# theovincent/iS-DQN

Hardware: AMD Instinct MI355X
Metric: gradient-steps/sec (batch=256, K=9, 84x84x4) (higher is better)
Workload: dtype bf16x3 (split-bf16 MFMA operands hi+lo, fp32 accumulate)

## Files before the change

is-dqn_amd/build.py:

```python
import os
import subprocess
import sys

HERE = os.path.dirname(os.path.abspath(__file__))
CSRC = os.path.join(HERE, "csrc")
LIBDIR = os.path.join(HERE, "lib")
LIB = os.path.join(LIBDIR, "libisdqn_hip.so")
SOURCES = ["api.hip", "tree_kernels.hip", "replay_kernels.hip", "net_kernels.hip"]
HEADERS = sorted(f for f in os.listdir(os.path.join(os.path.dirname(os.path.abspath(__file__)), "csrc")) if f.endswith(".h")) + [
    os.path.join("..", "..", "include", "isdqn_hip.h")]
FLAGS = ["--offload-arch=gfx950", "-O3", "-fPIC", "-std=c++17", "-fno-gpu-rdc", "-ffp-contract=off", "-fno-slp-vectorize"]


def _stale(target, deps):
    if not os.path.exists(target):
        return True
    t = os.path.getmtime(target)
    return any(os.path.getmtime(d) > t for d in deps)


def build(force=False, verbose=True, variant=None, defines=(), extra_flags=()):
    hipcc = os.environ.get("HIPCC", "/opt/rocm/bin/hipcc")
    os.makedirs(LIBDIR, exist_ok=True)
    objdir = os.path.join(HERE, "build" if not variant else "build_" + variant)
    lib = LIB if not variant else os.path.join(LIBDIR, "libisdqn_hip_%s.so" % variant)
    flags = FLAGS + ["-D" + d for d in defines] + list(extra_flags)
    os.makedirs(objdir, exist_ok=True)
    headers = [os.path.join(CSRC, h) for h in HEADERS]
    objs = []
    procs = []
    for src in SOURCES:
        s = os.path.join(CSRC, src)
        o = os.path.join(objdir, src.replace(".hip", ".o"))
        objs.append(o)
        if force or _stale(o, [s] + headers):
            cmd = [hipcc] + flags + ["-c", s, "-o", o]
            if verbose:
                print(" ".join(cmd), flush=True)
            procs.append((src, subprocess.Popen(cmd)))
    failed = [src for src, p in procs if p.wait() != 0]
    if failed:
        raise RuntimeError(f"hipcc failed for {failed}")
    if force or procs or _stale(lib, objs):
        cmd = [hipcc, "--offload-arch=gfx950", "-shared", "-fPIC", "-o", lib] + objs
        if verbose:
            print(" ".join(cmd), flush=True)
        subprocess.check_call(cmd)
    return lib


def emit_asm(force=False, verbose=False):
    hipcc = os.environ.get("HIPCC", "/opt/rocm/bin/hipcc")
    objdir = os.path.join(HERE, "build")
    os.makedirs(objdir, exist_ok=True)
    headers = [os.path.join(CSRC, h) for h in HEADERS]
    outs, procs = [], []
    for src in SOURCES:
        s = os.path.join(CSRC, src)
        o = os.path.join(objdir, src.replace(".hip", ".s"))
        outs.append(o)
        if force or _stale(o, [s] + headers + [os.path.abspath(__file__)]):
            cmd = [hipcc] + [f for f in FLAGS if f != "-fPIC"] + ["-S", "--cuda-device-only", "-w", s, "-o", o]
            if verbose:
                print(" ".join(cmd), flush=True)
            procs.append((src, subprocess.Popen(cmd)))
    failed = [src for src, p in procs if p.wait() != 0]
    if failed:
        raise RuntimeError(f"hipcc -S failed for {failed}")
    return outs


if __name__ == "__main__":
    _variant = None
    _defs = []
    for _i, _a in enumerate(sys.argv):
        if _a == "--variant":
            _variant = sys.argv[_i + 1]
        if _a.startswith("-D"):
            _defs.append(_a[2:])
    _extra = [_a for _a in sys.argv[1:] if _a.startswith("-f") or _a.startswith("-m")]
    print(build(force="--force" in sys.argv, variant=_variant, defines=_defs, extra_flags=_extra))
    if "--emit-asm" in sys.argv:
        print("\n".join(emit_asm(force="--force" in sys.argv, verbose=True)))
```

is-dqn_amd/csrc/conv_img.h:

```cpp
#pragma once
#include "net_problems.h"

namespace isdqn {

__device__ __forceinline__ int column_slot(int c16) { return c16 < 4 ? 8 + c16 : (c16 < 12 ? c16 - 4 : c16); }
struct PixelOrder {
    int strips;
    int n_full;
    int full_w;
    FastDiv d_h8, d_rem, d_w;
    PixelOrder() : strips(0), n_full(0), full_w(0) {}
    PixelOrder(int H, int W, bool use_strips) : strips(use_strips ? 1 : 0), n_full(H * 8 * (W / 8)), full_w(8 * (W / 8)) {
        d_h8 = FastDiv((uint32_t)(H * 8));
        d_rem = FastDiv((uint32_t)(W % 8 ? W % 8 : 1));
        d_w = FastDiv((uint32_t)W);
    }
    __device__ __forceinline__ void map(int n, int& y, int& x) const {
        uint32_t a, b;
        if (!strips) {
            d_w.divmod((uint32_t)n, a, b);
            y = (int)a; x = (int)b;
        } else if (n < n_full) {
            d_h8.divmod((uint32_t)n, a, b);
            y = (int)(b >> 3); x = (int)(a * 8 + (b & 7));
        } else {
            d_rem.divmod((uint32_t)(n - n_full), a, b);
            y = (int)a; x = full_w + (int)b;
        }
    }
};

struct ConvImgParams {
    ConvGeom g;
    MatSrc W;
    const float* in;
    FrameSrc fs;
    const float *bias, *gamma, *beta;
    float scale;
    float* act;
    float* z;
    int n_img, z_img;
    int tiles_per_img;
    int R, Wp;
    int PP;
    int plane_elems;
    int ablate;
    FastDiv d_chunk, d_Wp, d_R;
    PixelOrder order;
    long long* stamps;
};

template <int MT, int PASSES, bool U8>
struct ConvImgTraits {
    static constexpr int BM = MT * 16;
    static constexpr int A_PLANES = PASSES >= 2 ? 2 : 1;
    static constexpr int B_PLANES = (PASSES >= 3) ? 2 : 1;
    struct GA {
        static constexpr int PITCH = 48;
        static constexpr int ELEMS = BM * PITCH;
        static constexpr int CHUNKS = BM * (GEMM_BK / 8);
    };
    static constexpr int A_STAGE = A_PLANES * GA::ELEMS;
};

__device__ __forceinline__ void xcd_image_tile(int wg, int n_img, int T, int& j, int& tile) {
    const int full = (n_img / 8) * 8 * T;
    if (T > 1 && wg < full) {
        const int grp = wg / (8 * T), r = wg - grp * 8 * T;
        j = grp * 8 + (r & 7);
        tile = r >> 3;
    } else {
        j = wg / T;
        tile = wg - j * T;
    }
}

template <int NTHR, int PLANES, int BATCH>
__device__ __forceinline__ void fill_image_s8(__bf16* img, int plane_elems, const float* src, int H, int W, int C, int y0, int x0,
                                              int Rl, int Wl, int PP, int tid, const FastDiv& d_cpp, const FastDiv& d_Wl) {
    const int cpp = C >> 3, n_chunks = Rl * Wl * cpp;
    uint32_t pix_u, cc_u, lr_u, xl_u;
    d_cpp.divmod((uint32_t)tid, pix_u, cc_u);
    d_Wl.divmod(pix_u, lr_u, xl_u);
    int cc = (int)cc_u, lr = (int)lr_u, xl = (int)xl_u, pix = (int)pix_u;
    uint32_t dpix_u, dcc_u, dpy_u, dpx_u;
    d_cpp.divmod((uint32_t)NTHR, dpix_u, dcc_u);
    d_Wl.divmod(dpix_u, dpy_u, dpx_u);
    const int dpix = (int)dpix_u, dcc = (int)dcc_u, dpy = (int)dpy_u, dpx = (int)dpx_u;
    for (int c0 = tid; c0 - tid < n_chunks; ) {
        float v[BATCH][8];
        int dst[BATCH];
#pragma unroll
        for (int u = 0; u < BATCH; ++u) {
            const bool on = c0 < n_chunks;
            const int iy = y0 + lr, ix = x0 + xl;
            const bool ok = on && iy >= 0 && iy < H && ix >= 0 && ix < W;
            load8_aligned(ok ? src + ((iy * W + ix) * C + cc * 8) : zero_chunk(), v[u]);
            dst[u] = on ? pix * PP + cc * 8 : -1;
            c0 += NTHR;
            cc += dcc;
            const int carry_c = cc >= cpp ? 1 : 0;
            cc -= carry_c ? cpp : 0;
            pix += dpix + carry_c;
            xl += dpx + carry_c;
            lr += dpy;
            const int carry_x = xl >= Wl ? 1 : 0;
            xl -= carry_x ? Wl : 0;
            lr += carry_x;
        }
#pragma unroll
        for (int u = 0; u < BATCH; ++u) {
            bf16x8 hi, lo;
            if constexpr (PLANES >= 2) {
                s8_unpack(v[u], hi, lo);
                if (dst[u] >= 0) *reinterpret_cast<bf16x8*>(img + plane_elems + dst[u]) = lo;
            } else {
                s8_unpack_hi(v[u], hi);
            }
            if (dst[u] >= 0) *reinterpret_cast<bf16x8*>(img + dst[u]) = hi;
        }
    }
}

template <int N>
struct ImagePrefetch {
    float v[N][8];
    int dst[N];
};
template <int NTHR, int N>
__device__ __forceinline__ void request_image_s8(ImagePrefetch<N>& r, const float* src, int H, int W, int C, int y0, int x0, int Rl, int Wl,
                                                 int PP, int tid, const FastDiv& d_cpp, const FastDiv& d_Wl) {
    const int cpp = C >> 3, n_chunks = Rl * Wl * cpp;
    uint32_t pix_u, cc_u, lr_u, xl_u;
    d_cpp.divmod((uint32_t)tid, pix_u, cc_u);
    d_Wl.divmod(pix_u, lr_u, xl_u);
    int cc = (int)cc_u, lr = (int)lr_u, xl = (int)xl_u, pix = (int)pix_u;
    uint32_t dpix_u, dcc_u, dpy_u, dpx_u;
    d_cpp.divmod((uint32_t)NTHR, dpix_u, dcc_u);
    d_Wl.divmod(dpix_u, dpy_u, dpx_u);
    const int dpix = (int)dpix_u, dcc = (int)dcc_u, dpy = (int)dpy_u, dpx = (int)dpx_u;
    int c0 = tid;
#pragma unroll
    for (int u = 0; u < N; ++u) {
        const bool on = c0 < n_chunks;
        const int iy = y0 + lr, ix = x0 + xl;
        const bool ok = on && iy >= 0 && iy < H && ix >= 0 && ix < W;
        load8_aligned(ok ? src + ((iy * W + ix) * C + cc * 8) : zero_chunk(), r.v[u]);
        r.dst[u] = on ? pix * PP + cc * 8 : -1;
        c0 += NTHR;
        cc += dcc;
        const int carry_c = cc >= cpp ? 1 : 0;
        cc -= carry_c ? cpp : 0;
        pix += dpix + carry_c;
        xl += dpx + carry_c;
        lr += dpy;
        const int carry_x = xl >= Wl ? 1 : 0;
        xl -= carry_x ? Wl : 0;
        lr += carry_x;
    }
}
template <int PLANES, int N>
__device__ __forceinline__ void commit_image_s8(__bf16* img, int plane_elems, const ImagePrefetch<N>& r) {
#pragma unroll
    for (int u = 0; u < N; ++u) {
        bf16x8 hi, lo;
        if constexpr (PLANES >= 2) {
            s8_unpack(r.v[u], hi, lo);
            if (r.dst[u] >= 0) *reinterpret_cast<bf16x8*>(img + plane_elems + r.dst[u]) = lo;
        } else {
            s8_unpack_hi(r.v[u], hi);
        }
        if (r.dst[u] >= 0) *reinterpret_cast<bf16x8*>(img + r.dst[u]) = hi;
    }
}

template <int NTHR, int STACK_MAX = 4>
__device__ __forceinline__ void fill_frames_u8(__bf16* img, const FrameSrc& fs, int j, int row_base, int x0, int R, int Wp, int tid,
                                               const FastDiv& d_cpr) {
    constexpr int PB = 2;
    const int cpr = Wp / 8, per_plane = R * cpr, plane = R * Wp;
    const uint8_t* base[STACK_MAX];
#pragma unroll
    for (int c = 0; c < STACK_MAX; ++c) {
        const int id = c < fs.stack ? fs.frame_id(j, c) : -1;
        base[c] = id >= 0 ? fs.frames + (int64_t)id * fs.stride : nullptr;
    }
    const uint8_t* zeros = reinterpret_cast<const uint8_t*>(zero_chunk());
    for (int pb = 0; pb < per_plane; pb += NTHR * PB) {
        unsigned long long raw[PB][STACK_MAX];
        int sh[PB], dst[PB];
#pragma unroll
        for (int k = 0; k < PB; ++k) {
            const int pos = pb + k * NTHR + tid;
            const bool on = pos < per_plane;
            uint32_t lr, cx;
            d_cpr.divmod((uint32_t)(on ? pos : 0), lr, cx);
            const int iy = row_base + (int)lr, ix0 = (int)cx * 8 + x0;
            const bool ok = on && iy >= 0 && iy < fs.H && ix0 > -8 && ix0 < fs.W;
            const int ixc = min(max(ix0, 0), fs.W - 8);
            const int off = iy * fs.W + ixc;
            sh[k] = ix0 - ixc;
            dst[k] = on ? (int)lr * Wp + (int)cx * 8 : -1;
#pragma unroll
            for (int c = 0; c < STACK_MAX; ++c)
                raw[k][c] = load_u64_unaligned((ok && base[c] != nullptr) ? base[c] + off : zeros);
        }
#pragma unroll
        for (int k = 0; k < PB; ++k)
#pragma unroll
            for (int c = 0; c < STACK_MAX; ++c) {
                if (c >= fs.stack) continue;
                float v[8];
                FrameSrc::patch8_cvt(raw[k][c], sh[k], v);
                bf16x8 hi;
                round8(v, hi);
                if (dst[k] >= 0) *reinterpret_cast<bf16x8*>(img + c * plane + dst[k]) = hi;
            }
    }
}


template <int MT, int PASSES, bool U8, int KG = 1>
__global__ __launch_bounds__(GEMM_THREADS * KG, (U8 && MT == 2 && PASSES == 2) ? 4 : 1) void conv_fwd_img_kernel(const ConvImgParams p) {
    ISDQN_EMPTY_KERNEL_RETURN
    using T = ConvImgTraits<MT, PASSES, U8>;
    using GA = typename T::GA;
    constexpr int NT = 2;
    constexpr int NTHR = GEMM_THREADS;
    constexpr int NTHR_ALL = GEMM_THREADS * KG;
    constexpr int MTW = MT;
    extern __shared__ __attribute__((aligned(16))) char smem_raw[];
    __bf16* smem = reinterpret_cast<__bf16*>(smem_raw);
    const int tid_all = threadIdx.x, kg = KG > 1 ? tid_all / GEMM_THREADS : 0;
    __bf16* a_stage = smem + kg * 2 * T::A_STAGE;
    __bf16* img = smem + KG * 2 * T::A_STAGE;
    const ConvGeom& g = p.g;

    const int tid = tid_all - kg * GEMM_THREADS, lane = tid & 63, wave = tid >> 6;
#if defined(ISDQN_DEV)
#define ISDQN_STAMP(i)                                                                               \
    if (p.stamps != nullptr && threadIdx.x == 0) {                                                  \
        p.stamps[(int64_t)blockIdx.x * 8 + (i)] = (long long)__builtin_amdgcn_s_memtime();           \
        if ((i) == 0) p.stamps[(int64_t)blockIdx.x * 8 + 7] = (long long)__builtin_amdgcn_s_memrealtime(); \
    }
#define ISDQN_ABLATED(bit) ((p.ablate & (bit)) != 0)
#else
#define ISDQN_STAMP(i)
#define ISDQN_ABLATED(bit) (false)
#endif
    ISDQN_STAMP(0);
    if (ISDQN_ABLATED(8)) return;
    constexpr int mt0 = 0;
    int j, tile;
    xcd_image_tile((int)blockIdx.x, p.n_img, p.tiles_per_img, j, tile);
    const int p0 = tile * 128;
    const int oy_min = (int)g.d_wout.div((uint32_t)p0);
    const int row_base = oy_min * g.stride - g.pad;

    const int grp = lane >> 4;
    __shared__ __attribute__((aligned(16))) float s_par[3][64];
    float par_v = 0.f;
    {
        const int which = tid >> 6, ch = tid & 63;
        const float* src = which == 0 ? p.bias : which == 1 ? p.gamma : p.beta;
        const bool ok = kg == 0 && tid < 192 && ch < g.cout_p && src != nullptr;
        ISDQN_BOUNDS_CHECK(ok ? src + ch : zero_chunk(), 4, 13);
        par_v = *(const ISDQN_GLOBAL float*)(ok ? src + ch : zero_chunk());
    }

    const int nsteps = (g.K + GEMM_BK - 1) / GEMM_BK;
    const int k_last = g.K - 8;
    constexpr int A_PER = (GA::CHUNKS + NTHR - 1) / NTHR;
    int a_row[A_PER], a_var[A_PER], a_lds[A_PER];
    bool a_on[A_PER];
#pragma unroll
    for (int i = 0; i < A_PER; ++i) {
        int c = tid + i * NTHR;
        a_on[i] = c < GA::CHUNKS;
        if (!a_on[i]) c = 0;
        a_row[i] = stash_row(c);
        a_var[i] = (c & 3) * 8;
        a_lds[i] = a_row[i] * GA::PITCH + (c & 3) * 8;
    }
    constexpr int PF = 4;
    float sa[PF][A_PER][8];
    auto fetch = [&](int slot, int k) {
#pragma unroll
        for (int i = 0; i < A_PER; ++i) p.W.load(a_row[i], k + a_var[i], sa[slot][i]);
    };
    auto stash = [&](int slot, int stage) {
        __bf16* a_hi = a_stage + stage * T::A_STAGE;
        __bf16* a_lo = a_hi + GA::ELEMS;
#pragma unroll
        for (int i = 0; i < A_PER; ++i) {
            if (GA::CHUNKS % NTHR != 0 && !a_on[i]) continue;
            bf16x8 hi, lo;
            if constexpr (PASSES >= 2) {
                s8_unpack(sa[slot][i], hi, lo);
                *reinterpret_cast<bf16x8*>(a_lo + a_lds[i]) = lo;
            } else {
                s8_unpack_hi(sa[slot][i], hi);
            }
            *reinterpret_cast<bf16x8*>(a_hi + a_lds[i]) = hi;
        }
    };

    const int nsteps_p = ((nsteps + KG - 1) / KG + PF - 1) / PF * PF;
    const int rot = ISDQN_ABLATED(16) ? 0 : (int)((blockIdx.x >> 3) % (unsigned)nsteps);
    auto slice = [&](int s) {
        const int gs = s * KG + kg;
        const int k = gs + rot;
        return gs < nsteps ? (k >= nsteps ? k - nsteps : k) : nsteps_p * KG;
    };
#pragma unroll
    for (int d = 0; d < PF; ++d) fetch(d, slice(d) * GEMM_BK);

    constexpr int FILL_BATCH = (U8 ? 8 : 12) / KG;
    if (ISDQN_ABLATED(1)) {
    } else if constexpr (U8) {
#if defined(ISDQN_DEV)
        if (ISDQN_ABLATED(32)) {
            FrameSrc direct = p.fs;
            direct.ids = nullptr;
            fill_frames_u8<NTHR_ALL>(img, direct, j, row_base, -g.pad, p.R, p.Wp, tid_all, p.d_chunk);
        } else
#endif
        fill_frames_u8<NTHR_ALL>(img, p.fs, j, row_base, -g.pad, p.R, p.Wp, tid_all, p.d_chunk);
    } else {
        fill_image_s8<NTHR_ALL, T::B_PLANES, FILL_BATCH>(img, p.plane_elems, p.in + (int64_t)j * g.hin * g.win * g.cin_p, g.hin, g.win,
                                                         g.cin_p, row_base, -g.pad, p.R, p.Wp, p.PP, tid_all, p.d_chunk, p.d_Wp);
    }

    ISDQN_STAMP(1);
    int b_org[NT];
    int out_pix[NT];
#pragma unroll
    for (int nt = 0; nt < NT; ++nt) {
        int pp = p0 + wave * 32 + nt * 16 + (U8 ? (lane & 15) : column_slot(lane & 15));
        const bool in_img = pp < g.npix;
        pp = in_img ? pp : g.npix - 1;
        int oy, ox;
        if constexpr (U8) {
            uint32_t oy_u, ox_u;
            g.d_wout.divmod((uint32_t)pp, oy_u, ox_u);
            oy = (int)oy_u; ox = (int)ox_u;
        } else {
            p.order.map(pp, oy, ox);
        }
        out_pix[nt] = in_img ? oy * g.wout + ox : -1;
        const int ly0 = oy * g.stride - g.pad - row_base;
        const int lx0 = ox * g.stride;
        b_org[nt] = U8 ? (ly0 * p.Wp + lx0) : (ly0 * p.Wp + lx0) * p.PP;
    }

    f32x4 acc[MTW][NT];
#pragma unroll
    for (int mt = 0; mt < MTW; ++mt)
#pragma unroll
        for (int nt = 0; nt < NT; ++nt) mfma_init(acc[mt][nt]);


    struct Frags {
        bf16x8 a_hi[MTW], a_lo[MTW], b_hi[NT], b_lo[NT];
    };
    auto read_frags = [&](int stage, int kk, Frags& f) {
        const __bf16* a_hi = a_stage + stage * T::A_STAGE;
        const __bf16* a_lo = a_hi + GA::ELEMS;
#pragma unroll
        for (int mt = 0; mt < MTW; ++mt) {
            f.a_hi[mt] = read_frag<false, GA::PITCH>(a_hi, (mt0 + mt) * 16, lane);
            if constexpr (PASSES >= 2) f.a_lo[mt] = read_frag<false, GA::PITCH>(a_lo, (mt0 + mt) * 16, lane);
        }
        int kq = kk * GEMM_BK + grp * 8;
        kq = kq < k_last ? kq : k_last;
        int tap_off;
        if constexpr (U8) {
            const int c = kq >> 6, ky = (kq >> 3) & 7;
            tap_off = (c * p.R + ky) * p.Wp;
        } else {
            uint32_t tap, ci, ky, kx;
            g.d_cinp.divmod((uint32_t)kq, tap, ci);
            g.d_ksz.divmod(tap, ky, kx);
            tap_off = ((int)ky * p.Wp + (int)kx) * p.PP + (int)ci;
        }
#pragma unroll
        for (int nt = 0; nt < NT; ++nt) {
            const __bf16* src = img + b_org[nt] + tap_off;
            if constexpr (U8) {
                typedef __attribute__((ext_vector_type(4))) __bf16 bf16x4;
                bf16x4 h0 = *reinterpret_cast<const bf16x4*>(src);
                bf16x4 h1 = *reinterpret_cast<const bf16x4*>(src + 4);
                f.b_hi[nt] = __builtin_shufflevector(h0, h1, 0, 1, 2, 3, 4, 5, 6, 7);
            } else {
                f.b_hi[nt] = *reinterpret_cast<const bf16x8*>(src);
                if constexpr (PASSES >= 3) f.b_lo[nt] = *reinterpret_cast<const bf16x8*>(src + p.plane_elems);
            }
        }
    };
    auto mfma_step = [&](const Frags& f) {
#pragma unroll
        for (int nt = 0; nt < NT; ++nt)
#pragma unroll
            for (int mt = 0; mt < MTW; ++mt) {
                if constexpr (PASSES >= 3)
                    mfma_acc(acc[mt][nt], f.a_hi[mt], f.b_lo[nt]);
                if constexpr (PASSES >= 2)
                    mfma_acc(acc[mt][nt], f.a_lo[mt], f.b_hi[nt]);
                mfma_acc(acc[mt][nt], f.a_hi[mt], f.b_hi[nt]);
            }
    };

    static_assert(PF % 2 == 0 && PF >= 4, "the fragment sets alternate with the step parity; steps 0..3 are pre-fetched");
    Frags fr[2];
    if (kg == 0 && tid < 192) s_par[tid >> 6][tid & 63] = par_v;
    stash(0, 0);
    stash(1, 1);
    fetch(0, slice(PF) * GEMM_BK);
    fetch(1, slice(PF + 1) * GEMM_BK);
    __syncthreads();
    ISDQN_STAMP(2);
    if (!ISDQN_ABLATED(2)) {
        read_frags(0, slice(0), fr[0]);
        __syncthreads();
        constexpr bool INTERLEAVED = !U8 && PASSES == 3 && MTW == 4 && NT == 2 && A_PER == 1 &&
                                     GA::CHUNKS == NTHR;
        auto tap_offset_of = [&](int kk) {
            int kq = kk * GEMM_BK + grp * 8;
            kq = kq < k_last ? kq : k_last;
            uint32_t tap, ci, ky, kx;
            g.d_cinp.divmod((uint32_t)kq, tap, ci);
            g.d_ksz.divmod(tap, ky, kx);
            return ((int)ky * p.Wp + (int)kx) * p.PP + (int)ci;
        };
        int tap_next = INTERLEAVED ? tap_offset_of(slice(1)) : 0;
        for (int s0 = 0; s0 < nsteps_p; s0 += PF) {
#pragma unroll
            for (int u = 0; u < PF; ++u) {
                const int s = s0 + u;
                if constexpr (INTERLEAVED) {
                    const Frags& fc = fr[u & 1];
                    Frags& fn = fr[(u + 1) & 1];
                    const __bf16* na_hi = a_stage + ((s + 1) & 1) * T::A_STAGE;
                    const __bf16* na_lo = na_hi + GA::ELEMS;
                    const int tap_off = tap_next;
                    const int slot = (u + 2) % PF;
                    __bf16* st_hi = a_stage + (s & 1) * T::A_STAGE + a_lds[0];
                    __bf16* st_lo = st_hi + GA::ELEMS;
                    bf16x8 c_hi, c_lo;
                    __builtin_amdgcn_sched_barrier(0);
#pragma unroll
                    for (int j = 0; j < 24; ++j) {
                        const int pass = j >> 3, nt = (j >> 2) & 1, mt = j & 3;
                        mfma_acc(acc[mt][nt], pass == 1 ? fc.a_lo[mt] : fc.a_hi[mt], pass == 0 ? fc.b_lo[nt] : fc.b_hi[nt]);
                        if (j < 4) fn.a_hi[j] = read_frag<false, GA::PITCH>(na_hi, j * 16, lane);
                        else if (j < 8) fn.a_lo[j - 4] = read_frag<false, GA::PITCH>(na_lo, (j - 4) * 16, lane);
                        else if (j < 10) fn.b_hi[j - 8] = *reinterpret_cast<const bf16x8*>(img + b_org[j - 8] + tap_off);
                        else if (j < 12) fn.b_lo[j - 10] = *reinterpret_cast<const bf16x8*>(img + b_org[j - 10] + tap_off + p.plane_elems);
                        else if (j == 12) s8_unpack(sa[slot][0], c_hi, c_lo);
                        else if (j < 16) {
                        } else if (j == 16) *reinterpret_cast<bf16x8*>(st_lo) = c_lo;
                        else if (j == 17) *reinterpret_cast<bf16x8*>(st_hi) = c_hi;
                        else if (j == 18) fetch(slot, slice(s + 2 + PF) * GEMM_BK);
                        else if (j == 19) tap_next = tap_offset_of(slice(s + 2));
                        __builtin_amdgcn_sched_barrier(0);
                    }
                    __syncthreads();
                    continue;
                }
                read_frags((s + 1) & 1, slice(s + 1), fr[(u + 1) & 1]);
                mfma_step(fr[u & 1]);
                stash((u + 2) % PF, s & 1);
                fetch((u + 2) % PF, slice(s + 2 + PF) * GEMM_BK);
                constexpr int N_MFMA = MTW * NT * (PASSES >= 3 ? 3 : PASSES);
#pragma unroll
                for (int i = 0; i < N_MFMA; ++i) {
                    __builtin_amdgcn_sched_group_barrier(0x008, 1, 0);
                    if (i < N_MFMA / 2) __builtin_amdgcn_sched_group_barrier(0x100, 1, 0);
                    __builtin_amdgcn_sched_group_barrier(0x002, 2, 0);
                }
                __syncthreads();
            }
        }
    }
    ISDQN_STAMP(3);
    if constexpr (KG > 1) {
        static_assert(KG == 2 && NT == 2, "one pixel tile per K group");
        float* red = reinterpret_cast<float*>(img);
#pragma unroll
        for (int mt = 0; mt < MTW; ++mt)
#pragma unroll
            for (int r = 0; r < 4; ++r) {
                const float give = kg == 0 ? acc[mt][1][r] : acc[mt][0][r];
                red[(((kg * 4 + wave) * MTW + mt) * 4 + r) * 64 + lane] = give;
            }
        __syncthreads();
#pragma unroll
        for (int mt = 0; mt < MTW; ++mt)
#pragma unroll
            for (int r = 0; r < 4; ++r) {
                const float got = red[((((1 - kg) * 4 + wave) * MTW + mt) * 4 + r) * 64 + lane];
                if (kg == 0) acc[mt][0][r] += got;
                else acc[mt][1][r] += got;
            }
    }
    if (ISDQN_ABLATED(4)) {
        if (acc[0][0][0] == 12345.678f) p.act[0] = 1.f;
        return;
    }

    float bi[MTW][4], ga[MTW][4], be[MTW][4];
#pragma unroll
    for (int mt = 0; mt < MTW; ++mt) {
        const int ch0 = ((mt0 + mt) * 16 + grp * 4) & 63;
        const float4 b4 = *reinterpret_cast<const float4*>(&s_par[0][ch0]);
        const float4 g4 = *reinterpret_cast<const float4*>(&s_par[1][ch0]);
        const float4 e4 = *reinterpret_cast<const float4*>(&s_par[2][ch0]);
        bi[mt][0] = b4.x; bi[mt][1] = b4.y; bi[mt][2] = b4.z; bi[mt][3] = b4.w;
        ga[mt][0] = g4.x; ga[mt][1] = g4.y; ga[mt][2] = g4.z; ga[mt][3] = g4.w;
        be[mt][0] = e4.x; be[mt][1] = e4.y; be[mt][2] = e4.z; be[mt][3] = e4.w;
    }
    const float inv_c = 1.0f / (float)g.cout;
    float zv[NT][MTW][4], s1[NT], s2[NT];
#pragma unroll
    for (int nt = 0; nt < NT; ++nt) {
        s1[nt] = s2[nt] = 0.f;
        if (KG > 1 && nt != kg) continue;
#pragma unroll
        for (int mt = 0; mt < MTW; ++mt)
#pragma unroll
            for (int r = 0; r < 4; ++r) {
                int ch = (mt0 + mt) * 16 + grp * 4 + r;
                float zz = ch < g.cout ? acc[mt][nt][r] * p.scale + bi[mt][r] : 0.f;
                zv[nt][mt][r] = zz;
                s1[nt] += zz;
                s2[nt] += zz * zz;
            }
        if (p.gamma != nullptr) {
            s1[nt] += __shfl_xor(s1[nt], 16); s1[nt] += __shfl_xor(s1[nt], 32);
            s2[nt] += __shfl_xor(s2[nt], 16); s2[nt] += __shfl_xor(s2[nt], 32);
        }
    }
#pragma unroll
    for (int nt = 0; nt < NT; ++nt) {
        if (KG > 1 && nt != kg) continue;
        float mean = 0.f, rstd = 1.f;
        if (p.gamma != nullptr) {
            mean = s1[nt] * inv_c;
            float var = fmaxf(s2[nt] * inv_c - mean * mean, 0.f);
            rstd = rsqrtf(var + 1e-6f);
        }
        if (out_pix[nt] >= 0) {
            const int64_t pix = (int64_t)j * g.npix + out_pix[nt];
#pragma unroll
            for (int mt = 0; mt < MTW; ++mt) {
                int ch0 = (mt0 + mt) * 16 + grp * 4;
                if (ch0 >= g.cout_p) continue;
                float4 a, zq;
                float* ap = &a.x;
                float* zp = &zq.x;
#pragma unroll
                for (int r = 0; r < 4; ++r) {
                    float y = p.gamma != nullptr ? (zv[nt][mt][r] - mean) * (rstd * ga[mt][r]) + be[mt][r] : zv[nt][mt][r];
                    ap[r] = (ch0 + r < g.cout) ? fmaxf(y, 0.f) : 0.f;
                    zp[r] = zv[nt][mt][r];
                }
                s8_store_quad_paired(p.act + pix * g.cout_p, ch0, a.x, a.y, a.z, a.w);
                if (j < p.z_img) *reinterpret_cast<float4*>(p.z + pix * g.cout_p + ch0) = zq;
            }
        }
    }
    ISDQN_STAMP(4);
#if defined(ISDQN_DEV)
    if (p.stamps != nullptr) {
        __builtin_amdgcn_s_waitcnt(0);
        ISDQN_STAMP(5);
    }
#endif
#undef ISDQN_STAMP
#undef ISDQN_ABLATED
}

template <int MT, int PASSES, bool U8, int KG = 1>
static int launch_conv_fwd_img(const ConvImgParams& p, hipStream_t st) {
    using T = ConvImgTraits<MT, PASSES, U8>;
    const int lds = (KG * 2 * T::A_STAGE + T::B_PLANES * p.plane_elems) * 2;
    static LdsConfigured configured;
    if (int rc = ensure_dynamic_lds(&conv_fwd_img_kernel<MT, PASSES, U8, KG>, lds, configured)) return rc;
    ISDQN_REPORT_OCCUPANCY((&conv_fwd_img_kernel<MT, PASSES, U8, KG>), GEMM_THREADS * KG, lds, p.n_img * p.tiles_per_img);
    hipLaunchKernelGGL((conv_fwd_img_kernel<MT, PASSES, U8, KG>), dim3(p.n_img * p.tiles_per_img), dim3(GEMM_THREADS * KG), lds,
                       st, p);
    ISDQN_HIP_CHECK(hipGetLastError());
    return ISDQN_OK;
}

static inline int conv_img_geometry(const ConvGeom& g, bool u8, int stack, int b_planes, int mt, int a_planes, int& R,
                                    int& Wp, int& plane_elems, int pixel_pitch = 0) {
    int rows_per_tile = g.npix <= 128 ? g.hout : ((128 + g.wout - 2) / g.wout + 1);
    if (rows_per_tile > g.hout) rows_per_tile = g.hout;
    R = g.stride * (rows_per_tile - 1) + g.ksz;
    if (u8) {
        Wp = ((g.wout - 1) * g.stride + g.ksz + 7) / 8 * 8;
        plane_elems = stack * R * Wp;
    } else {
        Wp = (g.wout - 1) * g.stride + g.ksz;
        plane_elems = R * Wp * (pixel_pitch ? pixel_pitch : g.cin_p);
    }
    const int a_stage = a_planes * (mt * 16) * 48;
    return (2 * a_stage + b_planes * plane_elems) * 2;
}


struct ConvWgradImgParams {
    ConvGeom g;
    const float* dz;
    const float* in;
    FrameSrc fs;
    float* slabs;
    float scale;
    int n_img, G;
    int n_col_groups, NC;
    int R, Wp;
    int PPin;
    int in_plane;
    int PA, npix_pad;
    int dz_plane;
    FastDiv d_ncg;
    FastDiv d_chunk, d_Wp, d_R, d_dzchunk, d_npixpad;
    int prefetch;
    long long* stamps;
};
template <int WV> struct WgradPrefetch { static constexpr int DZ = 1024 / (64 * WV), IN = WV == 4 ? 6 : 5, DZ_U8 = 1792 / (64 * WV); };

template <bool U8, int PASSES, int NTHR = GEMM_THREADS>
__device__ __forceinline__ void fill_input_image(__bf16* img, int plane_elems, const ConvGeom& g, const FrameSrc& fs,
                                                 const float* in, int j, int row_base, int R, int Wp, int PP, int tid,
                                                 const FastDiv& d_chunk, const FastDiv& d_Wp, const FastDiv& d_R) {
    constexpr int FILL_BATCH = 8;
    if constexpr (U8) {
        fill_frames_u8<NTHR>(img, fs, j, row_base, -g.pad, R, Wp, tid, d_chunk);
    } else {
        fill_image_s8<NTHR, (PASSES >= 3 ? 2 : 1), FILL_BATCH>(img, plane_elems, in + (int64_t)j * g.hin * g.win * g.cin_p, g.hin, g.win, g.cin_p,
                                                               row_base, -g.pad, R, Wp, PP, tid, d_chunk, d_Wp);
    }
}

__device__ __forceinline__ bf16x8 tr_frag(const __bf16* a0, const __bf16* a1) {
    s16x4 lo = __builtin_amdgcn_ds_read_tr16_b64_v4i16((LDS_AS s16x4*)a0);
    s16x4 hi = __builtin_amdgcn_ds_read_tr16_b64_v4i16((LDS_AS s16x4*)a1);
    s16x8 r = __builtin_shufflevector(lo, hi, 0, 1, 2, 3, 4, 5, 6, 7);
    return __builtin_bit_cast(bf16x8, r);
}

template <int MT, int NTW, int PASSES, bool U8, int WV = 4>
__global__ __launch_bounds__(64 * WV) void conv_wgrad_img_kernel(const ConvWgradImgParams p) {
    ISDQN_EMPTY_KERNEL_RETURN
    constexpr int NTHR = 64 * WV;
    constexpr int A_PLANES = PASSES >= 2 ? 2 : 1;
    constexpr int B_PLANES = (PASSES >= 3) ? 2 : 1;
    extern __shared__ __attribute__((aligned(16))) char smem_raw[];
    __bf16* dzi = reinterpret_cast<__bf16*>(smem_raw);
    __bf16* img = dzi + A_PLANES * p.dz_plane;
    const ConvGeom& g = p.g;
    const int tid = threadIdx.x, lane = tid & 63, wave = tid >> 6;
#if defined(ISDQN_DEV)
#define WG_STAMP(i)                                                                                   \
    if (p.stamps != nullptr && threadIdx.x == 0) {                                                   \
        p.stamps[(int64_t)blockIdx.x * 8 + (i)] = (long long)__builtin_amdgcn_s_memtime();            \
        if ((i) == 0) p.stamps[(int64_t)blockIdx.x * 8 + 7] = (long long)__builtin_amdgcn_s_memrealtime(); \
    }
#else
#define WG_STAMP(i)
#endif
    WG_STAMP(0);
    uint32_t ig_u, cg_u;
    p.d_ncg.divmod(blockIdx.x, ig_u, cg_u);
    const int cg = (int)cg_u, ig = (int)ig_u;
    const int j0 = ig * p.G, j1 = min(p.n_img, j0 + p.G);
    const int grp = lane >> 4, li = lane & 15, q = li >> 2, pq = li & 3;

    int col_off[NTW];
#pragma unroll
    for (int t = 0; t < NTW; ++t) {
        const int c0 = cg * p.NC + (wave + WV * t) * 16;
        if constexpr (U8) {
            const int c = c0 >> 6, ky0 = (c0 >> 3) & 7;
            col_off[t] = (c * p.R + ky0 + (pq >> 1)) * p.Wp + 4 * (pq & 1);
        } else {
            uint32_t tap, ci, ky, kx;
            g.d_cinp.divmod((uint32_t)(c0 < g.K ? c0 : 0), tap, ci);
            g.d_ksz.divmod(tap, ky, kx);
            col_off[t] = ((int)ky * p.Wp + (int)kx) * p.PPin + (int)ci + 4 * pq;
        }
    }

    f32x4 acc[MT][NTW];
#pragma unroll
    for (int mt = 0; mt < MT; ++mt)
#pragma unroll
        for (int t = 0; t < NTW; ++t) mfma_init(acc[mt][t]);

    const int nsteps = p.npix_pad / GEMM_BK;
    auto k_steps = [&]() {
        for (int ks = 0; ks < nsteps; ++ks) {
            int pixoff[2], arow[2];
#pragma unroll
            for (int h = 0; h < 2; ++h) {
                int kp = ks * GEMM_BK + tr_row(8 * grp + 4 * h + q);
                arow[h] = kp * p.PA + 4 * pq;
                kp = kp < g.npix ? kp : g.npix - 1;
                uint32_t oy, ox;
                g.d_wout.divmod((uint32_t)kp, oy, ox);
                pixoff[h] = U8 ? ((int)oy * g.stride * p.Wp + (int)ox * g.stride)
                               : ((int)oy * g.stride * p.Wp + (int)ox * g.stride) * p.PPin;
            }
            bf16x8 fa_hi[MT], fa_lo[MT];
#pragma unroll
            for (int mt = 0; mt < MT; ++mt) {
                fa_hi[mt] = tr_frag(dzi + arow[0] + mt * 16, dzi + arow[1] + mt * 16);
                if constexpr (PASSES >= 2)
                    fa_lo[mt] = tr_frag(dzi + p.dz_plane + arow[0] + mt * 16, dzi + p.dz_plane + arow[1] + mt * 16);
            }
#pragma unroll
            for (int t = 0; t < NTW; ++t) {
                const __bf16* b0 = img + pixoff[0] + col_off[t];
                const __bf16* b1 = img + pixoff[1] + col_off[t];
                bf16x8 fb_hi = tr_frag(b0, b1), fb_lo;
                if constexpr (PASSES >= 3) fb_lo = tr_frag(b0 + p.in_plane, b1 + p.in_plane);
#pragma unroll
                for (int mt = 0; mt < MT; ++mt) {
                    if constexpr (PASSES >= 3)
                        mfma_acc(acc[mt][t], fa_hi[mt], fb_lo);
                    if constexpr (PASSES >= 2)
                        mfma_acc(acc[mt][t], fa_lo[mt], fb_hi);
                    mfma_acc(acc[mt][t], fa_hi[mt], fb_hi);
                }
            }
        }
    };
    bool staged = false;
    if constexpr (!U8) {
        if (p.prefetch) {
            staged = true;
            ImagePrefetch<WgradPrefetch<WV>::DZ> ra;
            ImagePrefetch<WgradPrefetch<WV>::IN> rb;
            auto request = [&](int j) {
                request_image_s8<NTHR>(ra, p.dz + (int64_t)j * g.npix * g.cout_p, 1, g.npix, g.cout_p, 0, 0, 1, p.npix_pad, p.PA, tid,
                                       p.d_dzchunk, p.d_npixpad);
                request_image_s8<NTHR>(rb, p.in + (int64_t)j * g.hin * g.win * g.cin_p, g.hin, g.win, g.cin_p, -g.pad, -g.pad, p.R, p.Wp,
                                       p.PPin, tid, p.d_chunk, p.d_Wp);
            };
            request(j0);
            for (int j = j0; j < j1; ++j) {
                __syncthreads();
                commit_image_s8<A_PLANES>(dzi, p.dz_plane, ra);
                commit_image_s8<B_PLANES>(img, p.in_plane, rb);
                __syncthreads();
                if (j == j0) { WG_STAMP(1); } else if (j == j0 + 1) { WG_STAMP(3); }
                if (j + 1 < j1) request(j + 1);
                k_steps();
                if (j == j0) { WG_STAMP(2); } else if (j == j0 + 1) { WG_STAMP(4); }
            }
        }
    }
    if (!staged)
    for (int j = j0; j < j1; ++j) {
        __syncthreads();
        bool dz_done = false;
        if constexpr (U8) {
            if (p.prefetch) {
                ImagePrefetch<WgradPrefetch<WV>::DZ_U8> ra;
                request_image_s8<NTHR>(ra, p.dz + (int64_t)j * g.npix * g.cout_p, 1, g.npix, g.cout_p, 0, 0, 1, p.npix_pad, p.PA, tid,
                                       p.d_dzchunk, p.d_npixpad);
                fill_input_image<U8, PASSES, NTHR>(img, p.in_plane, g, p.fs, p.in, j, -g.pad, p.R, p.Wp, p.PPin, tid, p.d_chunk, p.d_Wp, p.d_R);
                commit_image_s8<A_PLANES>(dzi, p.dz_plane, ra);
                dz_done = true;
            }
        }
        if (!dz_done) {
            fill_image_s8<NTHR, A_PLANES, 8>(dzi, p.dz_plane, p.dz + (int64_t)j * g.npix * g.cout_p, 1, g.npix, g.cout_p, 0, 0, 1, p.npix_pad,
                                             p.PA, tid, p.d_dzchunk, p.d_npixpad);
            fill_input_image<U8, PASSES, NTHR>(img, p.in_plane, g, p.fs, p.in, j, -g.pad, p.R, p.Wp, p.PPin, tid, p.d_chunk, p.d_Wp, p.d_R);
        }
        __syncthreads();
        if (j == j0) { WG_STAMP(1); } else if (j == j0 + 1) { WG_STAMP(3); }
        k_steps();
        if (j == j0) { WG_STAMP(2); } else if (j == j0 + 1) { WG_STAMP(4); }
    }

    float* slab = p.slabs + (int64_t)ig * g.cout_p * g.K;
#pragma unroll
    for (int mt = 0; mt < MT; ++mt)
#pragma unroll
        for (int t = 0; t < NTW; ++t) {
            const int col = cg * p.NC + (wave + WV * t) * 16 + li;
#pragma unroll
            for (int r = 0; r < 4; ++r) {
                const int row = mt * 16 + grp * 4 + r;
#if !defined(ISDQN_NO_STREAMING)
                if (row < g.cout_p && col < g.K) __builtin_nontemporal_store(acc[mt][t][r] * p.scale, (ISDQN_GLOBAL float*)(slab + (int64_t)row * g.K + col));
#else
                if (row < g.cout_p && col < g.K) slab[(int64_t)row * g.K + col] = acc[mt][t][r] * p.scale;
#endif
            }
        }
#if defined(ISDQN_DEV)
    if (p.stamps != nullptr) {
        __builtin_amdgcn_s_waitcnt(0);
        WG_STAMP(5);
    }
#endif
#undef WG_STAMP
}

template <int MT, int NTW, int PASSES, bool U8, int WV = 4>
static int launch_conv_wgrad_img(const ConvWgradImgParams& p, int n_img_groups, hipStream_t st) {
    constexpr int A_PLANES = PASSES >= 2 ? 2 : 1;
    constexpr int B_PLANES = (PASSES >= 3) ? 2 : 1;
    const int lds = (A_PLANES * p.dz_plane + B_PLANES * p.in_plane) * 2;
    static LdsConfigured configured;
    if (int rc = ensure_dynamic_lds(&conv_wgrad_img_kernel<MT, NTW, PASSES, U8, WV>, lds, configured)) return rc;
    ISDQN_REPORT_OCCUPANCY((&conv_wgrad_img_kernel<MT, NTW, PASSES, U8, WV>), 64 * WV, lds, n_img_groups * p.n_col_groups);
    ConvWgradImgParams q = p;
    q.prefetch = 0;
#if !defined(ISDQN_WGRAD_NO_PREFETCH)
    if (!U8 && p.G >= 2 && p.npix_pad * (p.g.cout_p / 8) <= WgradPrefetch<WV>::DZ * 64 * WV &&
        p.R * p.Wp * (p.g.cin_p / 8) <= WgradPrefetch<WV>::IN * 64 * WV)
        q.prefetch = 1;
#if !defined(ISDQN_WGRAD_NO_U8_DZ)
    if (U8 && p.npix_pad * (p.g.cout_p / 8) <= WgradPrefetch<WV>::DZ_U8 * 64 * WV) q.prefetch = 1;
#endif
#endif
    hipLaunchKernelGGL((conv_wgrad_img_kernel<MT, NTW, PASSES, U8, WV>), dim3(n_img_groups * p.n_col_groups),
                       dim3(64 * WV), lds, st, q);
    ISDQN_HIP_CHECK(hipGetLastError());
    return ISDQN_OK;
}


struct ConvDgradImgParams {
    ConvGeom g;
    const float* W;
    const float* dz;
    const float* z_in;
    const float *gamma, *beta;
    int c_in;
    float* dz_in;
    float* part;
    int n_img, T, Kc;
    int Hd, Wd, PPd, bt;
    FastDiv d_chunk, d_Wd, d_T;
    long long* stamps;
    int dz_plane;
    int tiles_per_img;
    int cls_tile_start[5];
    PixelOrder cls_order[4];
    int n_classes;
};

template <int MT, int PASSES, int NT = 2>
__global__ __launch_bounds__(GEMM_THREADS, 2) void conv_dgrad_img_kernel(const ConvDgradImgParams p) {
    ISDQN_EMPTY_KERNEL_RETURN
    constexpr int BM = MT * 16;
    constexpr int A_PLANES = PASSES >= 2 ? 2 : 1;
    constexpr int B_PLANES = PASSES >= 3 ? 2 : 1;
    using GA = TileGeom<BM, true>;
    constexpr int A_STAGE = A_PLANES * GA::ELEMS;
    extern __shared__ __attribute__((aligned(16))) char smem_raw[];
    __bf16* a_stage = reinterpret_cast<__bf16*>(smem_raw);
    __bf16* img = a_stage + 2 * A_STAGE;
    __shared__ float s_part[4][3][64];
    const ConvGeom& g = p.g;
    const int tid = threadIdx.x, lane = tid & 63, wave = tid >> 6, grp = lane >> 4;
#if defined(ISDQN_DEV)
#define ISDQN_STAMP(i)                                                                               \
    if (p.stamps != nullptr && threadIdx.x == 0) {                                                  \
        p.stamps[(int64_t)blockIdx.x * 8 + (i)] = (long long)__builtin_amdgcn_s_memtime();           \
        if ((i) == 0) p.stamps[(int64_t)blockIdx.x * 8 + 7] = (long long)__builtin_amdgcn_s_memrealtime(); \
    }
#define ISDQN_ABLATED(bit) ((p.ablate & (bit)) != 0)
#else
#define ISDQN_STAMP(i)
#define ISDQN_ABLATED(bit) (false)
#endif
    ISDQN_STAMP(0);

    int j, tl;
    xcd_image_tile((int)blockIdx.x, p.n_img, p.tiles_per_img, j, tl);
    int cls = 0;
    while (cls + 1 < p.n_classes && tl >= p.cls_tile_start[cls + 1]) ++cls;
    const int q0 = (tl - p.cls_tile_start[cls]) * (64 * NT);
    const int smask = g.stride - 1;
    const int cy = cls >> g.stride_sh, cx = cls & smask;
    const int Ha = (g.hin - cy + g.stride - 1) >> g.stride_sh, Wb = (g.win - cx + g.stride - 1) >> g.stride_sh;
    const int n_cls_pix = Ha * Wb;
    const int py = (cy + g.pad) & smask, px = (cx + g.pad) & smask;

    __shared__ __attribute__((aligned(16))) float s_gb[2][64];
    float par_v = 0.f;
    {
        const int which = tid >> 6, ch = tid & 63;
        const float* src = which == 0 ? p.gamma : p.beta;
        const bool ok = tid < 128 && ch < g.cin_p && p.gamma != nullptr;
        ISDQN_BOUNDS_CHECK(ok ? src + ch : zero_chunk(), 4, 13);
        par_v = *(const ISDQN_GLOBAL float*)(ok ? src + ch : zero_chunk());
    }

    const int nsteps = (p.Kc + GEMM_BK - 1) / GEMM_BK;
    const int k_last = p.Kc - 8;
    constexpr int A_PER = GA::PER_THREAD;
    int a_ci0[A_PER], a_kk[A_PER], a_lds[A_PER];
    bool a_on[A_PER];
#pragma unroll
    for (int i = 0; i < A_PER; ++i) {
        int c = tid + i * GEMM_THREADS;
        a_on[i] = c < GA::CHUNKS;
        if (!a_on[i]) c = 0;
        const int kk = c / (BM / 8), rc = c % (BM / 8);
        a_ci0[i] = rc * 8; a_kk[i] = kk;
        a_lds[i] = tr_row(kk) * GA::PITCH + rc * 8;
    }
    constexpr int PF = 4;
    float sa[PF][A_PER][8];
    auto fetch = [&](int slot, int k0) {
#pragma unroll
        for (int i = 0; i < A_PER; ++i) {
            const int k = k0 + a_kk[i];
            const bool ok = (k < p.Kc) && (a_ci0[i] < g.cin_p);
            uint32_t jt, co;
            g.d_coutp.divmod(ok ? (uint32_t)k : 0u, jt, co);
            uint32_t jy_u, jx_u;
            p.d_T.divmod(jt, jy_u, jx_u);
            const int jy = (int)jy_u, jx = (int)jx_u;
            const int ky = py + g.stride * jy, kx = px + g.stride * jx;
            load8_aligned(ok ? p.W + ((int64_t)co * g.K + (ky * g.ksz + kx) * g.cin_p + a_ci0[i]) : zero_chunk(), sa[slot][i]);
        }
    };
    auto stash = [&](int slot, int stage) {
        __bf16* a_hi = a_stage + stage * A_STAGE;
        __bf16* a_lo = a_hi + GA::ELEMS;
#pragma unroll
        for (int i = 0; i < A_PER; ++i) {
            if (GA::CHUNKS % GEMM_THREADS != 0 && !a_on[i]) continue;
            bf16x8 hi, lo;
            if constexpr (PASSES >= 2) {
                s8_unpack(sa[slot][i], hi, lo);
                *reinterpret_cast<bf16x8*>(a_lo + a_lds[i]) = lo;
            } else {
                s8_unpack_hi(sa[slot][i], hi);
            }
            *reinterpret_cast<bf16x8*>(a_hi + a_lds[i]) = hi;
        }
    };

    const int nsteps_p = (nsteps + PF - 1) / PF * PF;
    const int rot = (int)((blockIdx.x >> 3) % (unsigned)nsteps);
    auto slice = [&](int s) {
        const int k = s + rot;
        return s < nsteps ? (k >= nsteps ? k - nsteps : k) : nsteps_p;
    };
#pragma unroll
    for (int d = 0; d < PF; ++d) fetch(d, slice(d) * GEMM_BK);

    fill_image_s8<GEMM_THREADS, B_PLANES, 8>(img, p.dz_plane, p.dz + (int64_t)j * g.hout * g.wout * g.cout_p, g.hout, g.wout, g.cout_p,
                                             -p.bt, -p.bt, p.Hd, p.Wd, p.PPd, tid, p.d_chunk, p.d_Wd);

    ISDQN_STAMP(1);
    int b_org[NT], pix_iy[NT], pix_ix[NT];
    bool pix_ok[NT];
#pragma unroll
    for (int nt = 0; nt < NT; ++nt) {
        int q = q0 + wave * (16 * NT) + nt * 16 + column_slot(lane & 15);
        pix_ok[nt] = q < n_cls_pix;
        q = pix_ok[nt] ? q : n_cls_pix - 1;
        int a, b;
        p.cls_order[cls].map(q, a, b);
        const int iy = cy + g.stride * a, ix = cx + g.stride * b;
        pix_iy[nt] = iy; pix_ix[nt] = ix;
        const int oyb = (iy + g.pad - py) >> g.stride_sh, oxb = (ix + g.pad - px) >> g.stride_sh;
        b_org[nt] = ((oyb + p.bt) * p.Wd + oxb + p.bt) * p.PPd;
    }

    f32x4 acc[MT][NT];
#pragma unroll
    for (int mt = 0; mt < MT; ++mt)
#pragma unroll
        for (int nt = 0; nt < NT; ++nt) mfma_init(acc[mt][nt]);

    struct Frags {
        bf16x8 a_hi[MT], a_lo[MT], b_hi[NT], b_lo[NT];
    };
    auto read_frags = [&](int stage, int kk, Frags& f) {
        const __bf16* a_hi = a_stage + stage * A_STAGE;
        const __bf16* a_lo = a_hi + GA::ELEMS;
#pragma unroll
        for (int mt = 0; mt < MT; ++mt) {
            f.a_hi[mt] = read_frag<true, GA::PITCH>(a_hi, mt * 16, lane);
            if constexpr (PASSES >= 2) f.a_lo[mt] = read_frag<true, GA::PITCH>(a_lo, mt * 16, lane);
        }
        int kq = kk * GEMM_BK + grp * 8;
        kq = kq < k_last ? kq : k_last;
        uint32_t jt, co;
        g.d_coutp.divmod((uint32_t)kq, jt, co);
        uint32_t jy_u, jx_u;
        p.d_T.divmod(jt, jy_u, jx_u);
        const int jy = (int)jy_u, jx = (int)jx_u;
        const int tap_off = -(jy * p.Wd + jx) * p.PPd + (int)co;
#pragma unroll
        for (int nt = 0; nt < NT; ++nt) {
            const __bf16* src = img + b_org[nt] + tap_off;
            f.b_hi[nt] = *reinterpret_cast<const bf16x8*>(src);
            if constexpr (PASSES >= 3) f.b_lo[nt] = *reinterpret_cast<const bf16x8*>(src + p.dz_plane);
        }
    };
    auto mfma_step = [&](const Frags& f) {
#pragma unroll
        for (int nt = 0; nt < NT; ++nt)
#pragma unroll
            for (int mt = 0; mt < MT; ++mt) {
                if constexpr (PASSES >= 3)
                    mfma_acc(acc[mt][nt], f.a_hi[mt], f.b_lo[nt]);
                if constexpr (PASSES >= 2)
                    mfma_acc(acc[mt][nt], f.a_lo[mt], f.b_hi[nt]);
                mfma_acc(acc[mt][nt], f.a_hi[mt], f.b_hi[nt]);
            }
    };

    float zpre[NT][MT][4];
#pragma unroll
    for (int nt = 0; nt < NT; ++nt) {
        const int64_t pixel = ((int64_t)j * g.hin + pix_iy[nt]) * g.win + pix_ix[nt];
#pragma unroll
        for (int mt = 0; mt < MT; ++mt) {
            const int ch0 = mt * 16 + grp * 4;
            ISDQN_BOUNDS_CHECK(ch0 < g.cin_p ? p.z_in + pixel * g.cin_p + ch0 : zero_chunk(), 16, 12);
            const ISDQN_GLOBAL f32x4* zp = (const ISDQN_GLOBAL f32x4*)(ch0 < g.cin_p ? p.z_in + pixel * g.cin_p + ch0 : zero_chunk());
            const f32x4 zq = *zp;
            zpre[nt][mt][0] = zq[0]; zpre[nt][mt][1] = zq[1]; zpre[nt][mt][2] = zq[2]; zpre[nt][mt][3] = zq[3];
        }
    }

    static_assert(PF % 2 == 0 && PF >= 4, "the fragment sets alternate with the step parity; steps 0..3 are pre-fetched");
    Frags fr[2];
    if (tid < 128) s_gb[tid >> 6][tid & 63] = par_v;
    stash(0, 0);
    stash(1, 1);
    fetch(0, slice(PF) * GEMM_BK);
    fetch(1, slice(PF + 1) * GEMM_BK);
    __syncthreads();
    ISDQN_STAMP(2);
    read_frags(0, slice(0), fr[0]);
    __syncthreads();
    constexpr bool INTERLEAVED = PASSES == 3 && MT == 4 && A_PER == 1 && GA::CHUNKS == GEMM_THREADS;
    auto tap_offset_of = [&](int kk) {
        int kq = kk * GEMM_BK + grp * 8;
        kq = kq < k_last ? kq : k_last;
        uint32_t jt, co, jy_u, jx_u;
        g.d_coutp.divmod((uint32_t)kq, jt, co);
        p.d_T.divmod(jt, jy_u, jx_u);
        return -((int)jy_u * p.Wd + (int)jx_u) * p.PPd + (int)co;
    };
    int tap_next = INTERLEAVED ? tap_offset_of(slice(1)) : 0;
    for (int s0 = 0; s0 < nsteps_p; s0 += PF) {
#pragma unroll
        for (int u = 0; u < PF; ++u) {
            const int s = s0 + u;
            if constexpr (INTERLEAVED) {
                const Frags& fc = fr[u & 1];
                Frags& fn = fr[(u + 1) & 1];
                const __bf16* na_hi = a_stage + ((s + 1) & 1) * A_STAGE;
                const __bf16* na_lo = na_hi + GA::ELEMS;
                const int tap_off = tap_next;
                const int slot = (u + 2) % PF;
                __bf16* st_hi = a_stage + (s & 1) * A_STAGE + a_lds[0];
                __bf16* st_lo = st_hi + GA::ELEMS;
                bf16x8 c_hi, c_lo;
                constexpr int NM = 12 * NT;
                __builtin_amdgcn_sched_barrier(0);
#pragma unroll
                for (int jm = 0; jm < NM; ++jm) {
                    const int pass = jm / (4 * NT), nt = (jm >> 2) % NT, mt = jm & 3;
                    mfma_acc(acc[mt][nt], pass == 1 ? fc.a_lo[mt] : fc.a_hi[mt], pass == 0 ? fc.b_lo[nt] : fc.b_hi[nt]);
                    if (jm < 4) fn.a_hi[jm] = read_frag<true, GA::PITCH>(na_hi, jm * 16, lane);
                    else if (jm < 8) fn.a_lo[jm - 4] = read_frag<true, GA::PITCH>(na_lo, (jm - 4) * 16, lane);
                    else if (jm < 8 + NT) fn.b_hi[jm - 8] = *reinterpret_cast<const bf16x8*>(img + b_org[jm - 8] + tap_off);
                    else if (jm < 8 + 2 * NT) fn.b_lo[jm - 8 - NT] = *reinterpret_cast<const bf16x8*>(img + b_org[jm - 8 - NT] + tap_off + p.dz_plane);
                    else if constexpr (NT == 2) {
                        if (jm == 12) s8_unpack(sa[slot][0], c_hi, c_lo);
                        else if (jm == 16) *reinterpret_cast<bf16x8*>(st_lo) = c_lo;
                        else if (jm == 17) *reinterpret_cast<bf16x8*>(st_hi) = c_hi;
                        else if (jm == 18) fetch(slot, slice(s + 2 + PF) * GEMM_BK);
                        else if (jm == 19) tap_next = tap_offset_of(slice(s + 2));
                    } else {
                        if (jm == 10) {
                            s8_unpack(sa[slot][0], c_hi, c_lo);
                            *reinterpret_cast<bf16x8*>(st_lo) = c_lo;
                            *reinterpret_cast<bf16x8*>(st_hi) = c_hi;
                        } else if (jm == 11) {
                            fetch(slot, slice(s + 2 + PF) * GEMM_BK);
                            tap_next = tap_offset_of(slice(s + 2));
                        }
                    }
                    __builtin_amdgcn_sched_barrier(0);
                }
                __syncthreads();
                continue;
            }
            read_frags((s + 1) & 1, slice(s + 1), fr[(u + 1) & 1]);
            mfma_step(fr[u & 1]);
            stash((u + 2) % PF, s & 1);
            fetch((u + 2) % PF, slice(s + 2 + PF) * GEMM_BK);
            constexpr int N_MFMA = MT * NT * (PASSES >= 3 ? 3 : PASSES);
#pragma unroll
            for (int i = 0; i < N_MFMA; ++i) {
                __builtin_amdgcn_sched_group_barrier(0x008, 1, 0);
                if (i < N_MFMA / 2) __builtin_amdgcn_sched_group_barrier(0x100, 1, 0);
                __builtin_amdgcn_sched_group_barrier(0x002, 2, 0);
            }
            __syncthreads();
        }
    }

    ISDQN_STAMP(3);
    float ga[MT][4], be[MT][4];
#pragma unroll
    for (int mt = 0; mt < MT; ++mt) {
        const int ch0 = (mt * 16 + grp * 4) & 63;
        const float4 g4 = *reinterpret_cast<const float4*>(&s_gb[0][ch0]);
        const float4 e4 = *reinterpret_cast<const float4*>(&s_gb[1][ch0]);
        ga[mt][0] = g4.x; ga[mt][1] = g4.y; ga[mt][2] = g4.z; ga[mt][3] = g4.w;
        be[mt][0] = e4.x; be[mt][1] = e4.y; be[mt][2] = e4.z; be[mt][3] = e4.w;
    }
    float dg[MT][4], db[MT][4], dbias[MT][4];
#pragma unroll
    for (int mt = 0; mt < MT; ++mt)
#pragma unroll
        for (int r = 0; r < 4; ++r) dg[mt][r] = db[mt][r] = dbias[mt][r] = 0.f;
    const float inv_c = 1.f / (float)p.c_in;
#pragma unroll
    for (int nt = 0; nt < NT; ++nt) {
        const int64_t pixel = ((int64_t)j * g.hin + pix_iy[nt]) * g.win + pix_ix[nt];
        float zv[MT][4];
#pragma unroll
        for (int mt = 0; mt < MT; ++mt)
#pragma unroll
            for (int r = 0; r < 4; ++r) zv[mt][r] = zpre[nt][mt][r];
        float out[MT][4];
        if (p.gamma != nullptr) {
            float s1 = 0.f, s2 = 0.f;
#pragma unroll
            for (int mt = 0; mt < MT; ++mt)
#pragma unroll
                for (int r = 0; r < 4; ++r) {
                    const bool ok = (mt * 16 + grp * 4 + r) < p.c_in;
                    s1 += ok ? zv[mt][r] : 0.f;
                    s2 += ok ? zv[mt][r] * zv[mt][r] : 0.f;
                }
            s1 += __shfl_xor(s1, 16); s1 += __shfl_xor(s1, 32);
            s2 += __shfl_xor(s2, 16); s2 += __shfl_xor(s2, 32);
            const float mean = s1 * inv_c;
            const float rstd = rsqrtf(fmaxf(s2 * inv_c - mean * mean, 0.f) + 1e-6f);
            float xh[MT][4], gg[MT][4], m1 = 0.f, m2 = 0.f;
#pragma unroll
            for (int mt = 0; mt < MT; ++mt)
#pragma unroll
                for (int r = 0; r < 4; ++r) {
                    const bool ok = pix_ok[nt] && (mt * 16 + grp * 4 + r) < p.c_in;
                    xh[mt][r] = (zv[mt][r] - mean) * rstd;
                    const float y = xh[mt][r] * ga[mt][r] + be[mt][r];
                    const float dy = (ok && y > 0.f) ? acc[mt][nt][r] : 0.f;
                    dg[mt][r] += dy * xh[mt][r];
                    db[mt][r] += dy;
                    gg[mt][r] = dy * ga[mt][r];
                    m1 += gg[mt][r];
                    m2 += gg[mt][r] * xh[mt][r];
                }
            m1 += __shfl_xor(m1, 16); m1 += __shfl_xor(m1, 32);
            m2 += __shfl_xor(m2, 16); m2 += __shfl_xor(m2, 32);
            m1 *= inv_c;
            m2 *= inv_c;
#pragma unroll
            for (int mt = 0; mt < MT; ++mt)
#pragma unroll
                for (int r = 0; r < 4; ++r) {
                    const bool ok = pix_ok[nt] && (mt * 16 + grp * 4 + r) < p.c_in;
                    out[mt][r] = ok ? rstd * (gg[mt][r] - m1 - xh[mt][r] * m2) : 0.f;
                    dbias[mt][r] += out[mt][r];
                }
        } else {
#pragma unroll
            for (int mt = 0; mt < MT; ++mt)
#pragma unroll
                for (int r = 0; r < 4; ++r) {
                    const bool ok = pix_ok[nt] && (mt * 16 + grp * 4 + r) < p.c_in;
                    out[mt][r] = (ok && zv[mt][r] > 0.f) ? acc[mt][nt][r] : 0.f;
                    dbias[mt][r] += out[mt][r];
                }
        }
        if (pix_ok[nt]) {
#pragma unroll
            for (int mt = 0; mt < MT; ++mt) {
                const int ch0 = mt * 16 + grp * 4;
                if (ch0 < g.cin_p)
                    s8_store_quad_paired(p.dz_in + pixel * g.cin_p, ch0, out[mt][0], out[mt][1], out[mt][2], out[mt][3]);
            }
        }
    }
#pragma unroll
    for (int mt = 0; mt < MT; ++mt)
#pragma unroll
        for (int r = 0; r < 4; ++r) {
            dg[mt][r] = row16_sum(dg[mt][r]);
            db[mt][r] = row16_sum(db[mt][r]);
            dbias[mt][r] = row16_sum(dbias[mt][r]);
            if ((lane & 15) == 0) {
                const int ch = mt * 16 + grp * 4 + r;
                s_part[wave][0][ch] = dg[mt][r];
                s_part[wave][1][ch] = db[mt][r];
                s_part[wave][2][ch] = dbias[mt][r];
            }
        }
    __syncthreads();
    for (int i = tid; i < 3 * g.cin_p; i += GEMM_THREADS) {
        const int which = (i >= g.cin_p) + (i >= 2 * g.cin_p), c = i - which * g.cin_p;
        p.part[((int64_t)blockIdx.x * 3 + which) * g.cin_p + c] =
            s_part[0][which][c] + s_part[1][which][c] + s_part[2][which][c] + s_part[3][which][c];
    }
    ISDQN_STAMP(4);
#if defined(ISDQN_DEV)
    if (p.stamps != nullptr) {
        __builtin_amdgcn_s_waitcnt(0);
        ISDQN_STAMP(5);
    }
#endif
#undef ISDQN_STAMP
#undef ISDQN_ABLATED
}

constexpr int REDUCE_MAX_JOBS = 4;
struct ReduceJobs {
    const float* part[REDUCE_MAX_JOBS];
    float* out[REDUCE_MAX_JOBS];
    int n_rows[REDUCE_MAX_JOBS], width[REDUCE_MAX_JOBS];
    int block_start[REDUCE_MAX_JOBS + 1];
    int n;
};
__global__ __launch_bounds__(256) void reduce_rows_kernel(const ReduceJobs jobs) {
    ISDQN_EMPTY_KERNEL_RETURN
    __shared__ float s_red[32][8];
    int job = 0;
#pragma unroll
    for (int i = 1; i < REDUCE_MAX_JOBS; ++i)
        if (i < jobs.n && (int)blockIdx.x >= jobs.block_start[i]) job = i;
    const float* __restrict__ part = jobs.part[job];
    float* __restrict__ out = jobs.out[job];
    const int n_rows = jobs.n_rows[job], width = jobs.width[job];
    const int col = ((int)blockIdx.x - jobs.block_start[job]) * 8 + (threadIdx.x & 7), rl = threadIdx.x >> 3;
    float s = 0.f;
    if (col < width) {
        int r = rl;
        for (; r + 7 * 32 < n_rows; r += 8 * 32) {
            float v[8];
#pragma unroll
            for (int u = 0; u < 8; ++u) v[u] = part[(int64_t)(r + u * 32) * width + col];
#pragma unroll
            for (int u = 0; u < 8; ++u) s += v[u];
        }
        for (; r < n_rows; r += 32) s += part[(int64_t)r * width + col];
    }
    s_red[rl][threadIdx.x & 7] = s;
    __syncthreads();
    if (rl == 0 && col < width) {
        float t = 0.f;
#pragma unroll
        for (int k = 0; k < 32; ++k) t += s_red[k][threadIdx.x & 7];
        out[col] = t;
    }
}

template <int MT, int PASSES, int NT = 2>
static int launch_conv_dgrad_img(const ConvDgradImgParams& p, hipStream_t st) {
    constexpr int A_PLANES = PASSES >= 2 ? 2 : 1;
    constexpr int B_PLANES = PASSES >= 3 ? 2 : 1;
    using GA = TileGeom<MT * 16, true>;
    const int lds = (2 * A_PLANES * GA::ELEMS + B_PLANES * p.dz_plane) * 2;
    static LdsConfigured configured;
    if (int rc = ensure_dynamic_lds(&conv_dgrad_img_kernel<MT, PASSES, NT>, lds, configured)) return rc;
    ISDQN_REPORT_OCCUPANCY((&conv_dgrad_img_kernel<MT, PASSES, NT>), GEMM_THREADS, lds, p.n_img * p.tiles_per_img);
    hipLaunchKernelGGL((conv_dgrad_img_kernel<MT, PASSES, NT>), dim3(p.n_img * p.tiles_per_img), dim3(GEMM_THREADS), lds, st, p);
    ISDQN_HIP_CHECK(hipGetLastError());
    return ISDQN_OK;
}

}
```

is-dqn_amd/csrc/conv_s8_pair.h:

```cpp
#pragma once
#include "conv_img.h"

namespace isdqn {

constexpr int S8P_BATCH = 6;

template <int NPOS>
__global__ __launch_bounds__(GEMM_THREADS * 2, 1) void conv_fwd_s8_pair_kernel(const ConvImgParams p) {
    ISDQN_EMPTY_KERNEL_RETURN
    constexpr int MT = 4, PASSES = 3, KG = 2, NT = 2, MTW = MT, NTHR = GEMM_THREADS, NTHR_ALL = GEMM_THREADS * KG;
    using T = ConvImgTraits<MT, PASSES, false>;
    using GA = typename T::GA;
    extern __shared__ __attribute__((aligned(16))) char smem_raw[];
    __bf16* smem = reinterpret_cast<__bf16*>(smem_raw);
    const int tid_all = threadIdx.x, kg = tid_all / GEMM_THREADS;
    __bf16* a_stage = smem + kg * 2 * T::A_STAGE;
    __bf16* img = smem + KG * 2 * T::A_STAGE;
    const ConvGeom& g = p.g;
    const int tid = tid_all - kg * GEMM_THREADS, lane = tid & 63, wave = tid >> 6, grp = lane >> 4;
    const int row_base = -g.pad;

    __shared__ __attribute__((aligned(16))) float s_par[3][64];
    float par_v = 0.f;
    {
        const int which = tid >> 6, ch = tid & 63;
        const float* src = which == 0 ? p.bias : which == 1 ? p.gamma : p.beta;
        const bool ok = kg == 0 && tid < 192 && ch < g.cout_p && src != nullptr;
        ISDQN_BOUNDS_CHECK(ok ? src + ch : zero_chunk(), 4, 13);
        par_v = *(const ISDQN_GLOBAL float*)(ok ? src + ch : zero_chunk());
    }
    constexpr int nsteps = NPOS * KG;
    const int k_last = g.K - 8;
    static_assert(GA::CHUNKS == NTHR, "one weight chunk per thread and K step");
    const int a_row = stash_row(tid), a_var = (tid & 3) * 8, a_lds = a_row * GA::PITCH + (tid & 3) * 8;
    constexpr int PF = 4;
    static_assert(NPOS >= PF + 2, "ring of four slices + two staged ones");
    float sa[PF][1][8];
    auto fetch = [&](int slot, int k) { p.W.load(a_row, k + a_var, sa[slot][0]); };
    auto stash = [&](int slot, int stage) {
        __bf16* a_hi = a_stage + stage * T::A_STAGE;
        __bf16* a_lo = a_hi + GA::ELEMS;
        bf16x8 hi, lo;
        s8_unpack(sa[slot][0], hi, lo);
        *reinterpret_cast<bf16x8*>(a_lo + a_lds) = lo;
        *reinterpret_cast<bf16x8*>(a_hi + a_lds) = hi;
    };

    const int cpp = g.cin_p >> 3, n_chunks = p.R * p.Wp * cpp;
    uint32_t dpix_u, dcc_u, dpy_u, dpx_u;
    p.d_chunk.divmod((uint32_t)NTHR_ALL, dpix_u, dcc_u);
    p.d_Wp.divmod(dpix_u, dpy_u, dpx_u);
    const int dpix = (int)dpix_u, dcc = (int)dcc_u, dpy = (int)dpy_u, dpx = (int)dpx_u;
    float rv[S8P_BATCH][8];
    auto walk = [&](auto&& visit) {
        uint32_t pix_u, cc_u, lr_u, xl_u;
        p.d_chunk.divmod((uint32_t)tid_all, pix_u, cc_u);
        p.d_Wp.divmod(pix_u, lr_u, xl_u);
        int cc = (int)cc_u, lr = (int)lr_u, xl = (int)xl_u, pix = (int)pix_u, c0 = tid_all;
#pragma unroll
        for (int u = 0; u < S8P_BATCH; ++u) {
            visit(u, c0 < n_chunks, lr, xl, cc, pix);
            c0 += NTHR_ALL;
            cc += dcc;
            const int carry_c = cc >= cpp ? 1 : 0;
            cc -= carry_c ? cpp : 0;
            pix += dpix + carry_c;
            xl += dpx + carry_c;
            lr += dpy;
            const int carry_x = xl >= p.Wp ? 1 : 0;
            xl -= carry_x ? p.Wp : 0;
            lr += carry_x;
        }
    };
    auto request = [&](int j) {
        const float* src = p.in + (int64_t)j * g.hin * g.win * g.cin_p;
        walk([&](int u, bool on, int lr, int xl, int cc, int) {
            const int iy = row_base + lr, ix = xl - g.pad;
            const bool ok = on && iy >= 0 && iy < g.hin && ix >= 0 && ix < g.win;
            load8_aligned(ok ? src + ((iy * g.win + ix) * g.cin_p + cc * 8) : zero_chunk(), rv[u]);
        });
    };
    auto commit = [&]() {
        walk([&](int u, bool on, int, int, int cc, int pix) {
            bf16x8 hi, lo;
            s8_unpack(rv[u], hi, lo);
            if (on) {
                const int dst = pix * p.PP + cc * 8;
                *reinterpret_cast<bf16x8*>(img + p.plane_elems + dst) = lo;
                *reinterpret_cast<bf16x8*>(img + dst) = hi;
            }
        });
    };

    int b_org[NT], out_pix[NT];
#pragma unroll
    for (int nt = 0; nt < NT; ++nt) {
        int pp = wave * 32 + nt * 16 + column_slot(lane & 15);
        const bool in_img = pp < g.npix;
        pp = in_img ? pp : g.npix - 1;
        int oy, ox;
        p.order.map(pp, oy, ox);
        out_pix[nt] = in_img ? oy * g.wout + ox : -1;
        const int ly0 = oy * g.stride - g.pad - row_base;
        const int lx0 = ox * g.stride;
        b_org[nt] = (ly0 * p.Wp + lx0) * p.PP;
    }
    struct Frags {
        bf16x8 a_hi[MTW], a_lo[MTW], b_hi[NT], b_lo[NT];
    };

    auto do_image = [&](auto it_c) {
        constexpr int it = decltype(it_c)::value;
#if defined(ISDQN_PAIR_PLAIN_ORDER)
        const bool by_xcd = false;
#else
        const bool by_xcd = (p.n_img & 15) == 0;
#endif
        const int bx = (int)blockIdx.x;
        const int j_first = by_xcd ? ((bx >> 3) << 4) + (bx & 7) : 2 * bx;
        const int j_second = by_xcd ? j_first + 8 : j_first + 1;
        const int j = it == 0 ? j_first : j_second;
        const int rot = (int)((unsigned)(j >> 3) % (unsigned)nsteps);
        auto slice = [&](int s) {
            const int k = s * KG + kg + rot;
            return k >= nsteps ? k - nsteps : k;
        };
        auto tap_offset_of = [&](int kk) {
            int kq = kk * GEMM_BK + grp * 8;
            kq = kq < k_last ? kq : k_last;
            uint32_t tap, ci, ky, kx;
            g.d_cinp.divmod((uint32_t)kq, tap, ci);
            g.d_ksz.divmod(tap, ky, kx);
            return ((int)ky * p.Wp + (int)kx) * p.PP + (int)ci;
        };
#pragma unroll
        for (int d = 0; d < PF; ++d) fetch(d, slice(d) * GEMM_BK);
        if constexpr (it == 0) request(j);
        commit();

        f32x4 acc[MTW][NT];
#pragma unroll
        for (int mt = 0; mt < MTW; ++mt)
#pragma unroll
            for (int nt = 0; nt < NT; ++nt) mfma_init(acc[mt][nt]);
        Frags fr[2];
        if constexpr (it == 0) {
            if (kg == 0 && tid < 192) s_par[tid >> 6][tid & 63] = par_v;
        }
        stash(0, 0);
        stash(1, 1);
        fetch(0, slice(PF) * GEMM_BK);
        fetch(1, slice(PF + 1) * GEMM_BK);
        __syncthreads();
        {
            const __bf16* a_hi = a_stage;
            const __bf16* a_lo = a_hi + GA::ELEMS;
#pragma unroll
            for (int mt = 0; mt < MTW; ++mt) {
                fr[0].a_hi[mt] = read_frag<false, GA::PITCH>(a_hi, mt * 16, lane);
                fr[0].a_lo[mt] = read_frag<false, GA::PITCH>(a_lo, mt * 16, lane);
            }
            const int tap_off = tap_offset_of(slice(0));
#pragma unroll
            for (int nt = 0; nt < NT; ++nt) {
                const __bf16* src = img + b_org[nt] + tap_off;
                fr[0].b_hi[nt] = *reinterpret_cast<const bf16x8*>(src);
                fr[0].b_lo[nt] = *reinterpret_cast<const bf16x8*>(src + p.plane_elems);
            }
        }
        __syncthreads();
        int tap_next = tap_offset_of(slice(1));
#pragma unroll
        for (int s = 0; s < NPOS; ++s) {
            const Frags& fc = fr[s & 1];
            Frags& fn = fr[(s + 1) & 1];
            const __bf16* na_hi = a_stage + ((s + 1) & 1) * T::A_STAGE;
            const __bf16* na_lo = na_hi + GA::ELEMS;
            const int tap_off = tap_next;
            const int slot = (s + 2) % PF;
            __bf16* st_hi = a_stage + (s & 1) * T::A_STAGE + a_lds;
            __bf16* st_lo = st_hi + GA::ELEMS;
            const bool nxt = s + 1 < NPOS, stg = s + 2 < NPOS, ftc = s + 2 + PF < NPOS;
            bf16x8 c_hi, c_lo;
            __builtin_amdgcn_sched_barrier(0);
#pragma unroll
            for (int q = 0; q < 24; ++q) {
                const int pass = q >> 3, nt = (q >> 2) & 1, mt = q & 3;
                mfma_acc(acc[mt][nt], pass == 1 ? fc.a_lo[mt] : fc.a_hi[mt], pass == 0 ? fc.b_lo[nt] : fc.b_hi[nt]);
                if (q < 4) { if (nxt) fn.a_hi[q] = read_frag<false, GA::PITCH>(na_hi, q * 16, lane); }
                else if (q < 8) { if (nxt) fn.a_lo[q - 4] = read_frag<false, GA::PITCH>(na_lo, (q - 4) * 16, lane); }
                else if (q < 10) { if (nxt) fn.b_hi[q - 8] = *reinterpret_cast<const bf16x8*>(img + b_org[q - 8] + tap_off); }
                else if (q < 12) { if (nxt) fn.b_lo[q - 10] = *reinterpret_cast<const bf16x8*>(img + b_org[q - 10] + tap_off + p.plane_elems); }
                else if (q == 12) { if (stg) s8_unpack(sa[slot][0], c_hi, c_lo); }
                else if (q < 16) {
                } else if (q == 16) { if (stg) *reinterpret_cast<bf16x8*>(st_lo) = c_lo; }
                else if (q == 17) { if (stg) *reinterpret_cast<bf16x8*>(st_hi) = c_hi; }
                else if (q == 18) { if (ftc) fetch(slot, slice(s + 2 + PF) * GEMM_BK); }
                else if (q == 19) { if (s + 2 < NPOS) tap_next = tap_offset_of(slice(s + 2)); }
                __builtin_amdgcn_sched_barrier(0);
            }
            if constexpr (it == 0) {
                if (s == NPOS - 3) request(j_second);
            }
            __syncthreads();
        }
        {
            float* red = reinterpret_cast<float*>(img);
#pragma unroll
            for (int mt = 0; mt < MTW; ++mt)
#pragma unroll
                for (int r = 0; r < 4; ++r) {
                    const float give = kg == 0 ? acc[mt][1][r] : acc[mt][0][r];
                    red[(((kg * 4 + wave) * MTW + mt) * 4 + r) * 64 + lane] = give;
                }
            __syncthreads();
#pragma unroll
            for (int mt = 0; mt < MTW; ++mt)
#pragma unroll
                for (int r = 0; r < 4; ++r) {
                    const float got = red[((((1 - kg) * 4 + wave) * MTW + mt) * 4 + r) * 64 + lane];
                    if (kg == 0) acc[mt][0][r] += got;
                    else acc[mt][1][r] += got;
                }
        }
        float bi[MTW][4], ga[MTW][4], be[MTW][4];
#pragma unroll
        for (int mt = 0; mt < MTW; ++mt) {
            const int ch0 = (mt * 16 + grp * 4) & 63;
            const float4 b4 = *reinterpret_cast<const float4*>(&s_par[0][ch0]);
            const float4 g4 = *reinterpret_cast<const float4*>(&s_par[1][ch0]);
            const float4 e4 = *reinterpret_cast<const float4*>(&s_par[2][ch0]);
            bi[mt][0] = b4.x; bi[mt][1] = b4.y; bi[mt][2] = b4.z; bi[mt][3] = b4.w;
            ga[mt][0] = g4.x; ga[mt][1] = g4.y; ga[mt][2] = g4.z; ga[mt][3] = g4.w;
            be[mt][0] = e4.x; be[mt][1] = e4.y; be[mt][2] = e4.z; be[mt][3] = e4.w;
        }
        const float inv_c = 1.0f / (float)g.cout;
        float zv[NT][MTW][4], s1[NT], s2[NT];
#pragma unroll
        for (int nt = 0; nt < NT; ++nt) {
            s1[nt] = s2[nt] = 0.f;
            if (nt != kg) continue;
#pragma unroll
            for (int mt = 0; mt < MTW; ++mt)
#pragma unroll
                for (int r = 0; r < 4; ++r) {
                    int ch = mt * 16 + grp * 4 + r;
                    float zz = ch < g.cout ? acc[mt][nt][r] * p.scale + bi[mt][r] : 0.f;
                    zv[nt][mt][r] = zz;
                    s1[nt] += zz;
                    s2[nt] += zz * zz;
                }
            if (p.gamma != nullptr) {
                s1[nt] += __shfl_xor(s1[nt], 16); s1[nt] += __shfl_xor(s1[nt], 32);
                s2[nt] += __shfl_xor(s2[nt], 16); s2[nt] += __shfl_xor(s2[nt], 32);
            }
        }
#pragma unroll
        for (int nt = 0; nt < NT; ++nt) {
            if (nt != kg) continue;
            float mean = 0.f, rstd = 1.f;
            if (p.gamma != nullptr) {
                mean = s1[nt] * inv_c;
                float var = fmaxf(s2[nt] * inv_c - mean * mean, 0.f);
                rstd = rsqrtf(var + 1e-6f);
            }
            if (out_pix[nt] >= 0) {
                const int64_t pix = (int64_t)j * g.npix + out_pix[nt];
#pragma unroll
                for (int mt = 0; mt < MTW; ++mt) {
                    int ch0 = mt * 16 + grp * 4;
                    if (ch0 >= g.cout_p) continue;
                    float4 a, zq;
                    float* ap = &a.x;
                    float* zp = &zq.x;
#pragma unroll
                    for (int r = 0; r < 4; ++r) {
                        float y = p.gamma != nullptr ? (zv[nt][mt][r] - mean) * (rstd * ga[mt][r]) + be[mt][r] : zv[nt][mt][r];
                        ap[r] = (ch0 + r < g.cout) ? fmaxf(y, 0.f) : 0.f;
                        zp[r] = zv[nt][mt][r];
                    }
                    s8_store_quad_paired(p.act + pix * g.cout_p, ch0, a.x, a.y, a.z, a.w);
                    if (j < p.z_img) *reinterpret_cast<float4*>(p.z + pix * g.cout_p + ch0) = zq;
                }
            }
        }
        if constexpr (it == 0) __syncthreads();
    };
    do_image(std::integral_constant<int, 0>{});
    do_image(std::integral_constant<int, 1>{});
}

template <int NPOS>
static int launch_conv_fwd_s8_pair(const ConvImgParams& p, hipStream_t st) {
    using T = ConvImgTraits<4, 3, false>;
    const int lds = (2 * 2 * T::A_STAGE + T::B_PLANES * p.plane_elems) * 2;
    static LdsConfigured configured;
    if (int rc = ensure_dynamic_lds(&conv_fwd_s8_pair_kernel<NPOS>, lds, configured)) return rc;
    ISDQN_REPORT_OCCUPANCY((&conv_fwd_s8_pair_kernel<NPOS>), GEMM_THREADS * 2, lds, p.n_img / 2);
    hipLaunchKernelGGL((conv_fwd_s8_pair_kernel<NPOS>), dim3(p.n_img / 2), dim3(GEMM_THREADS * 2), lds, st, p);
    ISDQN_HIP_CHECK(hipGetLastError());
    return ISDQN_OK;
}

}
```

is-dqn_amd/csrc/conv_u8_pair.h:

```cpp
#pragma once
#include "conv_img.h"

namespace isdqn {

constexpr int U8P_PB = 2;

template <int PASSES, int NSTEPS>
__global__ __launch_bounds__(GEMM_THREADS, 4) void conv_fwd_u8_pair_kernel(const ConvImgParams p) {
    ISDQN_EMPTY_KERNEL_RETURN
    constexpr int MT = 2, NT = 2, MTW = MT, NTHR = GEMM_THREADS, STACK_MAX = 4;
    using T = ConvImgTraits<MT, PASSES, true>;
    using GA = typename T::GA;
    extern __shared__ __attribute__((aligned(16))) char smem_raw[];
    __bf16* smem = reinterpret_cast<__bf16*>(smem_raw);
    __bf16* a_stage = smem;
    __bf16* img = smem + 2 * T::A_STAGE;
    const ConvGeom& g = p.g;
    const int tid = threadIdx.x, lane = tid & 63, wave = tid >> 6, grp = lane >> 4;
#if defined(ISDQN_DEV)
#define U8P_STAMP(i)                                                                                 \
    if (p.stamps != nullptr && threadIdx.x == 0) {                                                  \
        p.stamps[(int64_t)blockIdx.x * 8 + (i)] = (long long)__builtin_amdgcn_s_memtime();           \
        if ((i) == 0) p.stamps[(int64_t)blockIdx.x * 8 + 7] = (long long)__builtin_amdgcn_s_memrealtime(); \
    }
#else
#define U8P_STAMP(i)
#endif
    U8P_STAMP(0);
    const int T2 = p.tiles_per_img >> 1;
    int j, tp;
    xcd_image_tile((int)blockIdx.x, p.n_img, T2, j, tp);

    __shared__ __attribute__((aligned(16))) float s_par[3][64];
    float par_v = 0.f;
    {
        const int which = tid >> 6, ch = tid & 63;
        const float* src = which == 0 ? p.bias : which == 1 ? p.gamma : p.beta;
        const bool ok = tid < 192 && ch < g.cout_p && src != nullptr;
        ISDQN_BOUNDS_CHECK(ok ? src + ch : zero_chunk(), 4, 13);
        par_v = *(const ISDQN_GLOBAL float*)(ok ? src + ch : zero_chunk());
    }
    constexpr int nsteps = NSTEPS;
    const int k_last = g.K - 8;
    constexpr int A_PER = (GA::CHUNKS + NTHR - 1) / NTHR;
    int a_row[A_PER], a_var[A_PER], a_lds[A_PER];
    bool a_on[A_PER];
#pragma unroll
    for (int i = 0; i < A_PER; ++i) {
        int c = tid + i * NTHR;
        a_on[i] = c < GA::CHUNKS;
        if (!a_on[i]) c = 0;
        a_row[i] = stash_row(c);
        a_var[i] = (c & 3) * 8;
        a_lds[i] = a_row[i] * GA::PITCH + (c & 3) * 8;
    }
    constexpr int PF = 4;
    float sa[PF][A_PER][8];
    auto fetch = [&](int slot, int k) {
#pragma unroll
        for (int i = 0; i < A_PER; ++i) p.W.load(a_row[i], k + a_var[i], sa[slot][i]);
    };
    auto stash = [&](int slot, int stage) {
        __bf16* a_hi = a_stage + stage * T::A_STAGE;
        __bf16* a_lo = a_hi + GA::ELEMS;
#pragma unroll
        for (int i = 0; i < A_PER; ++i) {
            if (GA::CHUNKS % NTHR != 0 && !a_on[i]) continue;
            bf16x8 hi, lo;
            if constexpr (PASSES >= 2) {
                s8_unpack(sa[slot][i], hi, lo);
                *reinterpret_cast<bf16x8*>(a_lo + a_lds[i]) = lo;
            } else {
                s8_unpack_hi(sa[slot][i], hi);
            }
            *reinterpret_cast<bf16x8*>(a_hi + a_lds[i]) = hi;
        }
    };
    static_assert(NSTEPS >= PF + 2 && NSTEPS % 2 == 0, "ring of four slices + two staged ones");

    const FrameSrc& fs = p.fs;
    const uint8_t* base[STACK_MAX];
#pragma unroll
    for (int c = 0; c < STACK_MAX; ++c) {
        const int id = c < fs.stack ? fs.frame_id(j, c) : -1;
        base[c] = id >= 0 ? fs.frames + (int64_t)id * fs.stride : nullptr;
    }
    const uint8_t* zeros = reinterpret_cast<const uint8_t*>(zero_chunk());
    const int cpr = p.Wp / 8, per_plane = p.R * cpr, plane = p.R * p.Wp;
    unsigned long long raw[U8P_PB][STACK_MAX];
    auto request = [&](int row_base) {
#pragma unroll
        for (int k = 0; k < U8P_PB; ++k) {
            const int pos = k * NTHR + tid;
            const bool on = pos < per_plane;
            uint32_t lr, cx;
            p.d_chunk.divmod((uint32_t)(on ? pos : 0), lr, cx);
            const int iy = row_base + (int)lr, ix0 = (int)cx * 8 - g.pad;
            const bool ok = on && iy >= 0 && iy < fs.H && ix0 > -8 && ix0 < fs.W;
            const int ixc = min(max(ix0, 0), fs.W - 8);
            const int off = iy * fs.W + ixc;
#pragma unroll
            for (int c = 0; c < STACK_MAX; ++c) raw[k][c] = load_u64_unaligned((ok && base[c] != nullptr) ? base[c] + off : zeros);
        }
    };
    auto commit = [&]() {
#pragma unroll
        for (int k = 0; k < U8P_PB; ++k) {
            const int pos = k * NTHR + tid;
            const bool on = pos < per_plane;
            uint32_t lr, cx;
            p.d_chunk.divmod((uint32_t)(on ? pos : 0), lr, cx);
            const int ix0 = (int)cx * 8 - g.pad;
            const int sh = ix0 - min(max(ix0, 0), fs.W - 8);
            const int dst = (int)lr * p.Wp + (int)cx * 8;
#pragma unroll
            for (int c = 0; c < STACK_MAX; ++c) {
                if (c >= fs.stack) continue;
                float v[8];
                FrameSrc::patch8_cvt(raw[k][c], sh, v);
                bf16x8 hi;
                round8(v, hi);
                if (on) *reinterpret_cast<bf16x8*>(img + c * plane + dst) = hi;
            }
        }
    };
    auto tile_rows = [&](int tile) {
        const int oy_min = (int)g.d_wout.div((uint32_t)(tile * 128));
        return oy_min * g.stride - g.pad;
    };

    struct Frags {
        bf16x8 a_hi[MTW], a_lo[MTW], b_hi[NT];
    };

    auto do_tile = [&](auto it_c) {
        constexpr int it = decltype(it_c)::value;
        const int tile = 2 * tp + it;
        const int p0 = tile * 128;
        const int row_base = tile_rows(tile);
        const int full = (p.n_img / 8) * 8;
        const int old_wg8 = j < full ? (j >> 3) * p.tiles_per_img + tile : (j * p.tiles_per_img + tile) >> 3;
        const int rot = (int)((unsigned)old_wg8 % (unsigned)nsteps);
        auto slice = [&](int s) {
            const int k = s + rot;
            return k >= nsteps ? k - nsteps : k;
        };
#pragma unroll
        for (int d = 0; d < PF; ++d) fetch(d, slice(d) * GEMM_BK);
        if constexpr (it == 0) request(row_base);
        commit();
        U8P_STAMP(it == 0 ? 1 : 4);

        int b_org[NT], out_pix[NT];
#pragma unroll
        for (int nt = 0; nt < NT; ++nt) {
            int pp = p0 + wave * 32 + nt * 16 + (lane & 15);
            const bool in_img = pp < g.npix;
            pp = in_img ? pp : g.npix - 1;
            uint32_t oy_u, ox_u;
            g.d_wout.divmod((uint32_t)pp, oy_u, ox_u);
            const int oy = (int)oy_u, ox = (int)ox_u;
            out_pix[nt] = in_img ? oy * g.wout + ox : -1;
            const int ly0 = oy * g.stride - g.pad - row_base;
            const int lx0 = ox * g.stride;
            b_org[nt] = ly0 * p.Wp + lx0;
        }
        f32x4 acc[MTW][NT];
#pragma unroll
        for (int mt = 0; mt < MTW; ++mt)
#pragma unroll
            for (int nt = 0; nt < NT; ++nt) mfma_init(acc[mt][nt]);

        auto read_frags = [&](int stage, int kk, Frags& f) {
            const __bf16* a_hi = a_stage + stage * T::A_STAGE;
            const __bf16* a_lo = a_hi + GA::ELEMS;
#pragma unroll
            for (int mt = 0; mt < MTW; ++mt) {
                f.a_hi[mt] = read_frag<false, GA::PITCH>(a_hi, mt * 16, lane);
                if constexpr (PASSES >= 2) f.a_lo[mt] = read_frag<false, GA::PITCH>(a_lo, mt * 16, lane);
            }
            int kq = kk * GEMM_BK + grp * 8;
            kq = kq < k_last ? kq : k_last;
            const int c = kq >> 6, ky = (kq >> 3) & 7;
            const int tap_off = (c * p.R + ky) * p.Wp;
#pragma unroll
            for (int nt = 0; nt < NT; ++nt) {
                const __bf16* src = img + b_org[nt] + tap_off;
                typedef __attribute__((ext_vector_type(4))) __bf16 bf16x4;
                bf16x4 h0 = *reinterpret_cast<const bf16x4*>(src);
                bf16x4 h1 = *reinterpret_cast<const bf16x4*>(src + 4);
                f.b_hi[nt] = __builtin_shufflevector(h0, h1, 0, 1, 2, 3, 4, 5, 6, 7);
            }
        };
        auto mfma_step = [&](const Frags& f) {
#pragma unroll
            for (int nt = 0; nt < NT; ++nt)
#pragma unroll
                for (int mt = 0; mt < MTW; ++mt) {
                    if constexpr (PASSES >= 2) mfma_acc(acc[mt][nt], f.a_lo[mt], f.b_hi[nt]);
                    mfma_acc(acc[mt][nt], f.a_hi[mt], f.b_hi[nt]);
                }
        };
        Frags fr[2];
        if constexpr (it == 0) {
            if (tid < 192) s_par[tid >> 6][tid & 63] = par_v;
        }
        stash(0, 0);
        stash(1, 1);
        fetch(0, slice(PF) * GEMM_BK);
        fetch(1, slice(PF + 1) * GEMM_BK);
        __syncthreads();
        read_frags(0, slice(0), fr[0]);
        __syncthreads();
#pragma unroll
        for (int s = 0; s < NSTEPS; ++s) {
            if (s + 1 < NSTEPS) read_frags((s + 1) & 1, slice(s + 1), fr[(s + 1) & 1]);
            mfma_step(fr[s & 1]);
            if (s + 2 < NSTEPS) stash((s + 2) % PF, s & 1);
            if (s + 2 + PF < NSTEPS) fetch((s + 2) % PF, slice(s + 2 + PF) * GEMM_BK);
            if constexpr (it == 0) {
                if (s == NSTEPS - 3) request(tile_rows(tile + 1));
            }
            constexpr int N_MFMA = MTW * NT * (PASSES >= 3 ? 3 : PASSES);
#pragma unroll
            for (int i = 0; i < N_MFMA; ++i) {
                __builtin_amdgcn_sched_group_barrier(0x008, 1, 0);
                if (i < N_MFMA / 2) __builtin_amdgcn_sched_group_barrier(0x100, 1, 0);
                __builtin_amdgcn_sched_group_barrier(0x002, 2, 0);
            }
            __syncthreads();
        }

        U8P_STAMP(it == 0 ? 2 : 5);
        float bi[MTW][4], ga[MTW][4], be[MTW][4];
#pragma unroll
        for (int mt = 0; mt < MTW; ++mt) {
            const int ch0 = (mt * 16 + grp * 4) & 63;
            const float4 b4 = *reinterpret_cast<const float4*>(&s_par[0][ch0]);
            const float4 g4 = *reinterpret_cast<const float4*>(&s_par[1][ch0]);
            const float4 e4 = *reinterpret_cast<const float4*>(&s_par[2][ch0]);
            bi[mt][0] = b4.x; bi[mt][1] = b4.y; bi[mt][2] = b4.z; bi[mt][3] = b4.w;
            ga[mt][0] = g4.x; ga[mt][1] = g4.y; ga[mt][2] = g4.z; ga[mt][3] = g4.w;
            be[mt][0] = e4.x; be[mt][1] = e4.y; be[mt][2] = e4.z; be[mt][3] = e4.w;
        }
        const float inv_c = 1.0f / (float)g.cout;
        float zv[NT][MTW][4], s1[NT], s2[NT];
#pragma unroll
        for (int nt = 0; nt < NT; ++nt) {
            s1[nt] = s2[nt] = 0.f;
#pragma unroll
            for (int mt = 0; mt < MTW; ++mt)
#pragma unroll
                for (int r = 0; r < 4; ++r) {
                    int ch = mt * 16 + grp * 4 + r;
                    float zz = ch < g.cout ? acc[mt][nt][r] * p.scale + bi[mt][r] : 0.f;
                    zv[nt][mt][r] = zz;
                    s1[nt] += zz;
                    s2[nt] += zz * zz;
                }
            if (p.gamma != nullptr) {
                s1[nt] += __shfl_xor(s1[nt], 16); s1[nt] += __shfl_xor(s1[nt], 32);
                s2[nt] += __shfl_xor(s2[nt], 16); s2[nt] += __shfl_xor(s2[nt], 32);
            }
        }
#pragma unroll
        for (int nt = 0; nt < NT; ++nt) {
            float mean = 0.f, rstd = 1.f;
            if (p.gamma != nullptr) {
                mean = s1[nt] * inv_c;
                float var = fmaxf(s2[nt] * inv_c - mean * mean, 0.f);
                rstd = rsqrtf(var + 1e-6f);
            }
            if (out_pix[nt] >= 0) {
                const int64_t pix = (int64_t)j * g.npix + out_pix[nt];
#pragma unroll
                for (int mt = 0; mt < MTW; ++mt) {
                    int ch0 = mt * 16 + grp * 4;
                    if (ch0 >= g.cout_p) continue;
                    float4 a, zq;
                    float* ap = &a.x;
                    float* zp = &zq.x;
#pragma unroll
                    for (int r = 0; r < 4; ++r) {
                        float y = p.gamma != nullptr ? (zv[nt][mt][r] - mean) * (rstd * ga[mt][r]) + be[mt][r] : zv[nt][mt][r];
                        ap[r] = (ch0 + r < g.cout) ? fmaxf(y, 0.f) : 0.f;
                        zp[r] = zv[nt][mt][r];
                    }
                    s8_store_quad_paired(p.act + pix * g.cout_p, ch0, a.x, a.y, a.z, a.w);
                    if (j < p.z_img) *reinterpret_cast<float4*>(p.z + pix * g.cout_p + ch0) = zq;
                }
            }
        }
        U8P_STAMP(it == 0 ? 3 : 6);
    };
    do_tile(std::integral_constant<int, 0>{});
    do_tile(std::integral_constant<int, 1>{});
#undef U8P_STAMP
}

template <int PASSES, int NSTEPS>
static int launch_conv_fwd_u8_pair(const ConvImgParams& p, hipStream_t st) {
    using T = ConvImgTraits<2, PASSES, true>;
    const int lds = (2 * T::A_STAGE + T::B_PLANES * p.plane_elems) * 2;
    static LdsConfigured configured;
    if (int rc = ensure_dynamic_lds(&conv_fwd_u8_pair_kernel<PASSES, NSTEPS>, lds, configured)) return rc;
    const int grid = p.n_img * (p.tiles_per_img / 2);
    ISDQN_REPORT_OCCUPANCY((&conv_fwd_u8_pair_kernel<PASSES, NSTEPS>), GEMM_THREADS, lds, grid);
    hipLaunchKernelGGL((conv_fwd_u8_pair_kernel<PASSES, NSTEPS>), dim3(grid), dim3(GEMM_THREADS), lds, st, p);
    ISDQN_HIP_CHECK(hipGetLastError());
    return ISDQN_OK;
}

}
```

is-dqn_amd/csrc/gemm_core.h:

```cpp
#pragma once
#include <cstdio>
#include <cstdlib>
#include <type_traits>
#include "common.h"

namespace isdqn {

typedef __attribute__((ext_vector_type(8))) __bf16 bf16x8;
typedef __attribute__((ext_vector_type(4))) short s16x4;
typedef __attribute__((ext_vector_type(8))) short s16x8;
typedef __attribute__((ext_vector_type(4))) float f32x4;

constexpr int GEMM_BK = 32;
constexpr int GEMM_THREADS = 256;

__device__ __forceinline__ int xcd_remap(int bid, int n_blocks) {
    const int xcd = bid & 7, q = n_blocks >> 3, r = n_blocks & 7;
    const int base = xcd < r ? xcd * (q + 1) : r * (q + 1) + (xcd - r) * q;
    return base + (bid >> 3);
}

#define LDS_AS __attribute__((address_space(3)))

__device__ __forceinline__ void split8(const float (&v)[8], bf16x8& hi, bf16x8& lo) {
#pragma unroll
    for (int i = 0; i < 8; ++i) {
        __bf16 h = (__bf16)v[i];
        hi[i] = h;
        lo[i] = (__bf16)(v[i] - (float)h);
    }
}
__device__ __forceinline__ void round8(const float (&v)[8], bf16x8& hi) {
#pragma unroll
    for (int i = 0; i < 8; ++i) hi[i] = (__bf16)v[i];
}

__device__ __forceinline__ void s8_unpack(const float (&raw)[8], bf16x8& hi, bf16x8& lo) {
    const f32x4 h = {raw[0], raw[1], raw[2], raw[3]}, l = {raw[4], raw[5], raw[6], raw[7]};
    hi = __builtin_bit_cast(bf16x8, h);
    lo = __builtin_bit_cast(bf16x8, l);
}
__device__ __forceinline__ void s8_unpack_hi(const float (&raw)[8], bf16x8& hi) {
    const f32x4 h = {raw[0], raw[1], raw[2], raw[3]};
    hi = __builtin_bit_cast(bf16x8, h);
}
template <bool S8>
__device__ __forceinline__ void chunk_planes(const float (&v)[8], bf16x8& hi, bf16x8& lo) {
    if constexpr (S8) s8_unpack(v, hi, lo);
    else split8(v, hi, lo);
}
template <bool S8>
__device__ __forceinline__ void chunk_hi(const float (&v)[8], bf16x8& hi) {
    if constexpr (S8) s8_unpack_hi(v, hi);
    else round8(v, hi);
}
__device__ __forceinline__ void s8_store_group(float* group, const float (&v)[8]) {
    bf16x8 hi, lo;
    split8(v, hi, lo);
    reinterpret_cast<bf16x8*>(group)[0] = hi;
    reinterpret_cast<bf16x8*>(group)[1] = lo;
}
__device__ __forceinline__ void s8_store_quad(float* row, int c0, float v0, float v1, float v2, float v3) {
    typedef __attribute__((ext_vector_type(4))) __bf16 bf16x4;
    const float v[4] = {v0, v1, v2, v3};
    bf16x4 hi, lo;
#pragma unroll
    for (int i = 0; i < 4; ++i) {
        const __bf16 h = (__bf16)v[i];
        hi[i] = h;
        lo[i] = (__bf16)(v[i] - (float)h);
    }
    char* g = reinterpret_cast<char*>(row + (c0 & ~7)) + (c0 & 4) * 2;
    *reinterpret_cast<bf16x4*>(g) = hi;
    *reinterpret_cast<bf16x4*>(g + 16) = lo;
}

__device__ __forceinline__ void s8_store_quad_paired(float* row, int c0, float v0, float v1, float v2, float v3) {
    typedef __attribute__((ext_vector_type(4))) __bf16 bf16x4;
    typedef __attribute__((ext_vector_type(2))) unsigned u32x2;
    typedef __attribute__((ext_vector_type(4))) unsigned u32x4;
    const float v[4] = {v0, v1, v2, v3};
    bf16x4 hi, lo;
#pragma unroll
    for (int i = 0; i < 4; ++i) {
        const __bf16 h = (__bf16)v[i];
        hi[i] = h;
        lo[i] = (__bf16)(v[i] - (float)h);
    }
    const u32x2 h = __builtin_bit_cast(u32x2, hi), l = __builtin_bit_cast(u32x2, lo);
    const auto r0 = __builtin_amdgcn_permlane16_swap(h[0], l[0], false, false);
    const auto r1 = __builtin_amdgcn_permlane16_swap(h[1], l[1], false, false);
    char* g = reinterpret_cast<char*>(row + (c0 & ~7)) + (c0 & 4) * 4;
    *reinterpret_cast<u32x4*>(g) = u32x4{r0[0], r1[0], r0[1], r1[1]};
}

__device__ __forceinline__ void s8_store_pair(float* row, int c0, float v0, float v1) {
    typedef __attribute__((ext_vector_type(2))) __bf16 bf16x2;
    const __bf16 h0 = (__bf16)v0, h1 = (__bf16)v1;
    char* g = reinterpret_cast<char*>(row + (c0 & ~7)) + (c0 & 7) * 2;
    *reinterpret_cast<bf16x2*>(g) = bf16x2{h0, h1};
    *reinterpret_cast<bf16x2*>(g + 16) = bf16x2{(__bf16)(v0 - (float)h0), (__bf16)(v1 - (float)h1)};
}
__device__ __forceinline__ void s8_store_elem(float* row, int c, float v) {
    const __bf16 h = (__bf16)v;
    __bf16* g = reinterpret_cast<__bf16*>(row + (c & ~7)) + (c & 7);
    g[0] = h;
    g[8] = (__bf16)(v - (float)h);
}

__device__ __forceinline__ constexpr int stash_row(int chunk) {
    return ((chunk >> 4) << 2) + (((chunk >> 2) & 1) << 1) + ((chunk >> 3) & 1);
}
__device__ __forceinline__ constexpr int tr_row(int kk) {
    return 16 * (kk >> 4) + 8 * ((kk >> 2) & 1) + 2 * (kk & 3) + ((kk >> 3) & 1);
}
template <int ROWS, bool TR, int TR_PAD = 16>
struct TileGeom {
    static constexpr int PITCH = TR ? (ROWS + TR_PAD) : (GEMM_BK + 16);
    static constexpr int ELEMS = TR ? GEMM_BK * PITCH : ROWS * PITCH;
    static constexpr int CHUNKS = ROWS * (GEMM_BK / 8);
    static constexpr int PER_THREAD = (CHUNKS + GEMM_THREADS - 1) / GEMM_THREADS;
};

__device__ __forceinline__ void mfma_init(f32x4& acc) { acc = f32x4{0.f, 0.f, 0.f, 0.f}; }
__device__ __forceinline__ void mfma_acc(f32x4& acc, const bf16x8& a, const bf16x8& b) {
    acc = __builtin_amdgcn_mfma_f32_16x16x32_bf16(a, b, acc, 0, 0, 0);
}

template <bool TR, int PITCH>
__device__ __forceinline__ bf16x8 read_frag(const __bf16* tile, int row0, int lane) {
    if constexpr (!TR) {
        return *reinterpret_cast<const bf16x8*>(tile + (row0 + (lane & 15)) * PITCH + (lane >> 4) * 8);
    } else {
        const int g = lane >> 4, i = lane & 15, q = i >> 2, p = i & 3;
        const __bf16* a0 = tile + (16 * (g >> 1) + 2 * q + (g & 1)) * PITCH + row0 + 4 * p;
        const __bf16* a1 = a0 + 8 * PITCH;
        s16x4 lo = __builtin_amdgcn_ds_read_tr16_b64_v4i16((LDS_AS s16x4*)a0);
        s16x4 hi = __builtin_amdgcn_ds_read_tr16_b64_v4i16((LDS_AS s16x4*)a1);
        s16x8 r = __builtin_shufflevector(lo, hi, 0, 1, 2, 3, 4, 5, 6, 7);
        return __builtin_bit_cast(bf16x8, r);
    }
}

template <class P, class = void>
struct KGroupsOf { static constexpr int value = 1; };
template <class P>
struct KGroupsOf<P, std::void_t<decltype(P::KG)>> { static constexpr int value = P::KG; };
template <class P, class = void>
struct TrPadAOf { static constexpr int value = 16; };
template <class P>
struct TrPadAOf<P, std::void_t<decltype(P::TR_PAD_A)>> { static constexpr int value = P::TR_PAD_A; };
template <class P, class = void>
struct TrPadBOf { static constexpr int value = 16; };
template <class P>
struct TrPadBOf<P, std::void_t<decltype(P::TR_PAD_B)>> { static constexpr int value = P::TR_PAD_B; };
template <class P, class = void>
struct AS8Of { static constexpr bool value = false; };
template <class P>
struct AS8Of<P, std::void_t<decltype(P::A_S8)>> { static constexpr bool value = P::A_S8; };
template <class P, class = void>
struct BS8Of { static constexpr bool value = false; };
template <class P>
struct BS8Of<P, std::void_t<decltype(P::B_S8)>> { static constexpr bool value = P::B_S8; };

template <class P>
struct GemmTraits {
    static constexpr int BM = P::BM, BN = P::BN, WM = P::WM, WN = P::WN;
    static constexpr int MT = BM / WM / 16, NT = BN / WN / 16;
    static constexpr int PASSES = P::PASSES;
    static constexpr int A_PLANES = PASSES >= 2 ? 2 : 1;
    static constexpr int B_PLANES = PASSES >= 3 ? 2 : 1;
    using GA = TileGeom<BM, P::A_TR, TrPadAOf<P>::value>;
    using GB = TileGeom<BN, P::B_TR, TrPadBOf<P>::value>;
    static constexpr int STAGE_ELEMS = A_PLANES * GA::ELEMS + B_PLANES * GB::ELEMS;
    static constexpr int KG = KGroupsOf<P>::value;
    static constexpr int PIPE_BYTES = KG * 2 * STAGE_ELEMS * 2;
    static constexpr int XCHG_BYTES = KG > 1 ? KG * 4 * NT * 4 * 64 * 4 : 0;
    static constexpr int EPI_BYTES = P::EPI_LDS_BYTES + XCHG_BYTES;
    static constexpr int LDS_BYTES = PIPE_BYTES > EPI_BYTES ? PIPE_BYTES : EPI_BYTES;
};

template <class P>
__global__ __launch_bounds__(GEMM_THREADS * KGroupsOf<P>::value) void gemm_kernel(const P p) {
    ISDQN_EMPTY_KERNEL_RETURN
    using T = GemmTraits<P>;
    constexpr int KG = T::KG;
    using GA = typename T::GA;
    using GB = typename T::GB;
    constexpr int MT = T::MT, NT = T::NT, PASSES = T::PASSES;
    extern __shared__ __attribute__((aligned(16))) char smem_raw[];
    __bf16* smem = reinterpret_cast<__bf16*>(smem_raw);

    typename P::Tile tile;
    if (!p.tile((int)blockIdx.x, tile)) return;

    const int kg = KG > 1 ? (int)threadIdx.x / GEMM_THREADS : 0;
    const int tid = (int)threadIdx.x - kg * GEMM_THREADS;
    const int lane = tid & 63;
    const int wave = tid >> 6;
    const int wm = wave / P::WN, wn = wave % P::WN;
    const int wave_m = wm * (MT * 16), wave_n = wn * (NT * 16);

    typename P::ACtx actx[GA::PER_THREAD];
    typename P::BCtx bctx[GB::PER_THREAD];
    int a_lds[GA::PER_THREAD], a_var[GA::PER_THREAD];
    int b_lds[GB::PER_THREAD], b_var[GB::PER_THREAD];
    bool a_on[GA::PER_THREAD], b_on[GB::PER_THREAD];
#pragma unroll
    for (int i = 0; i < GA::PER_THREAD; ++i) {
        int c = tid + i * GEMM_THREADS;
        a_on[i] = c < GA::CHUNKS;
        if (!a_on[i]) c = 0;
        if constexpr (!P::A_TR) {
            int r = stash_row(c), kc = c & 3;
            actx[i] = p.a_ctx(tile, tile.m0 + r);
            a_var[i] = kc * 8;
            a_lds[i] = r * GA::PITCH + kc * 8;
        } else {
            int kk = c / (T::BM / 8), rc = c % (T::BM / 8);
            actx[i] = p.a_ctx(tile, tile.m0 + rc * 8);
            a_var[i] = kk;
            a_lds[i] = tr_row(kk) * GA::PITCH + rc * 8;
        }
    }
#pragma unroll
    for (int i = 0; i < GB::PER_THREAD; ++i) {
        int c = tid + i * GEMM_THREADS;
        b_on[i] = c < GB::CHUNKS;
        if (!b_on[i]) c = 0;
        if constexpr (!P::B_TR) {
            int r = stash_row(c), kc = c & 3;
            bctx[i] = p.b_ctx(tile, tile.n0 + r);
            b_var[i] = kc * 8;
            b_lds[i] = r * GB::PITCH + kc * 8;
        } else {
            int kk = c / (T::BN / 8), rc = c % (T::BN / 8);
            bctx[i] = p.b_ctx(tile, tile.n0 + rc * 8);
            b_var[i] = kk;
            b_lds[i] = tr_row(kk) * GB::PITCH + rc * 8;
        }
    }

    float sa[GA::PER_THREAD][8], sb[GB::PER_THREAD][8];

    auto fetch = [&](int k) {
#pragma unroll
        for (int i = 0; i < GA::PER_THREAD; ++i)
            if (GA::CHUNKS % GEMM_THREADS == 0 || a_on[i]) p.load_a(tile, actx[i], k + a_var[i], sa[i]);
#pragma unroll
        for (int i = 0; i < GB::PER_THREAD; ++i)
            if (GB::CHUNKS % GEMM_THREADS == 0 || b_on[i]) p.load_b(tile, bctx[i], k + b_var[i], sb[i]);
    };
    auto stash = [&](int stage) {
        __bf16* base = smem + (kg * 2 + stage) * T::STAGE_ELEMS;
        __bf16* a_hi = base;
        __bf16* a_lo = base + GA::ELEMS;
        __bf16* b_hi = base + T::A_PLANES * GA::ELEMS;
        __bf16* b_lo = b_hi + GB::ELEMS;
#pragma unroll
        for (int i = 0; i < GA::PER_THREAD; ++i) {
            if (GA::CHUNKS % GEMM_THREADS != 0 && !a_on[i]) continue;
            bf16x8 hi, lo;
            if constexpr (PASSES >= 2) {
                chunk_planes<AS8Of<P>::value>(sa[i], hi, lo);
                *reinterpret_cast<bf16x8*>(a_lo + a_lds[i]) = lo;
            } else {
                chunk_hi<AS8Of<P>::value>(sa[i], hi);
            }
            *reinterpret_cast<bf16x8*>(a_hi + a_lds[i]) = hi;
        }
#pragma unroll
        for (int i = 0; i < GB::PER_THREAD; ++i) {
            if (GB::CHUNKS % GEMM_THREADS != 0 && !b_on[i]) continue;
            bf16x8 hi, lo;
            if constexpr (PASSES >= 3) {
                chunk_planes<BS8Of<P>::value>(sb[i], hi, lo);
                *reinterpret_cast<bf16x8*>(b_lo + b_lds[i]) = lo;
            } else {
                chunk_hi<BS8Of<P>::value>(sb[i], hi);
            }
            *reinterpret_cast<bf16x8*>(b_hi + b_lds[i]) = hi;
        }
    };

    f32x4 acc[MT][NT];
#pragma unroll
    for (int mt = 0; mt < MT; ++mt)
#pragma unroll
        for (int nt = 0; nt < NT; ++nt) mfma_init(acc[mt][nt]);

    auto compute = [&](int stage) {
        const __bf16* base = smem + (kg * 2 + stage) * T::STAGE_ELEMS;
        const __bf16* a_hi = base;
        const __bf16* a_lo = base + GA::ELEMS;
        const __bf16* b_hi = base + T::A_PLANES * GA::ELEMS;
        const __bf16* b_lo = b_hi + GB::ELEMS;
        bf16x8 fa_hi[MT], fa_lo[MT];
#pragma unroll
        for (int mt = 0; mt < MT; ++mt) {
            fa_hi[mt] = read_frag<P::A_TR, GA::PITCH>(a_hi, wave_m + mt * 16, lane);
            if constexpr (PASSES >= 2) fa_lo[mt] = read_frag<P::A_TR, GA::PITCH>(a_lo, wave_m + mt * 16, lane);
        }
#pragma unroll
        for (int nt = 0; nt < NT; ++nt) {
            bf16x8 fb_hi = read_frag<P::B_TR, GB::PITCH>(b_hi, wave_n + nt * 16, lane);
            bf16x8 fb_lo;
            if constexpr (PASSES >= 3) fb_lo = read_frag<P::B_TR, GB::PITCH>(b_lo, wave_n + nt * 16, lane);
#pragma unroll
            for (int mt = 0; mt < MT; ++mt) {
                if constexpr (PASSES >= 3)
                    mfma_acc(acc[mt][nt], fa_hi[mt], fb_lo);
                if constexpr (PASSES >= 2)
                    mfma_acc(acc[mt][nt], fa_lo[mt], fb_hi);
                mfma_acc(acc[mt][nt], fa_hi[mt], fb_hi);
            }
        }
    };

    const int nsteps = ((tile.k1 - tile.k0 + GEMM_BK - 1) / GEMM_BK + KG - 1) / KG;
    if (nsteps > 0) {
        fetch(tile.k0 + kg * GEMM_BK);
        stash(0);
        __syncthreads();
        for (int s = 0; s < nsteps; ++s) {
            const bool more = s + 1 < nsteps;
            if (more) fetch(tile.k0 + ((s + 1) * KG + kg) * GEMM_BK);
            compute(s & 1);
            if (more) stash((s + 1) & 1);
            __syncthreads();
        }
    }
    if constexpr (KG > 1) {
        static_assert(KG == 2 && MT == 2, "one row tile per K group");
        float* red = reinterpret_cast<float*>(smem_raw + P::EPI_LDS_BYTES);
#pragma unroll
        for (int nt = 0; nt < NT; ++nt)
#pragma unroll
            for (int r = 0; r < 4; ++r) {
                const float give = kg == 0 ? acc[1][nt][r] : acc[0][nt][r];
                red[(((kg * 4 + wave) * NT + nt) * 4 + r) * 64 + lane] = give;
            }
        __syncthreads();
        f32x4 mine[1][NT];
#pragma unroll
        for (int nt = 0; nt < NT; ++nt)
#pragma unroll
            for (int r = 0; r < 4; ++r) {
                const float got = red[((((1 - kg) * 4 + wave) * NT + nt) * 4 + r) * 64 + lane];
                mine[0][nt][r] = (kg == 0 ? acc[0][nt][r] : acc[1][nt][r]) + got;
            }
        p.epilogue(tile, mine, tile.m0 + wave_m + kg * 16, tile.n0 + wave_n, lane, smem_raw);
    } else {
        p.epilogue(tile, acc, tile.m0 + wave_m, tile.n0 + wave_n, lane, smem_raw);
    }
}

template <class P>
static int launch_gemm(const P& p, int n_blocks, hipStream_t stream) {
    using T = GemmTraits<P>;
    static LdsConfigured configured;
    int rc = ensure_dynamic_lds(&gemm_kernel<P>, T::LDS_BYTES, configured);
    if (rc) return rc;
    ISDQN_REPORT_OCCUPANCY((&gemm_kernel<P>), GEMM_THREADS * T::KG, T::LDS_BYTES, n_blocks);
    if (n_blocks <= 0) return ISDQN_OK;
    hipLaunchKernelGGL(gemm_kernel<P>, dim3(n_blocks), dim3(GEMM_THREADS * T::KG), T::LDS_BYTES, stream, p);
    ISDQN_HIP_CHECK(hipGetLastError());
    return ISDQN_OK;
}

__device__ __forceinline__ void zero8(float (&v)[8]) {
#pragma unroll
    for (int i = 0; i < 8; ++i) v[i] = 0.f;
}
__device__ __forceinline__ float row16_sum(float x) {
    auto dpp = [](float v, auto ctrl) {
        return __builtin_bit_cast(float, __builtin_amdgcn_update_dpp(0, __builtin_bit_cast(int, v), decltype(ctrl)::value, 0xF, 0xF, true));
    };
    x += dpp(x, std::integral_constant<int, 0xB1>{});
    x += dpp(x, std::integral_constant<int, 0x4E>{});
    x += dpp(x, std::integral_constant<int, 0x124>{});
    x += dpp(x, std::integral_constant<int, 0x128>{});
    return x;
}

static __device__ const float isdqn_zero_block[16] = {0.f, 0.f, 0.f, 0.f, 0.f, 0.f, 0.f, 0.f,
                                                      0.f, 0.f, 0.f, 0.f, 0.f, 0.f, 0.f, 0.f};
__device__ __forceinline__ const float* zero_chunk() { return isdqn_zero_block; }

#if defined(ISDQN_BOUNDS)
struct BoundsTable {
    int n, bad, bad_site, pad;
    unsigned long long bad_addr;
    unsigned long long lo[64], hi[64];
};
static __device__ BoundsTable isdqn_bounds;
__device__ __forceinline__ void bounds_check(const void* p, int bytes, int site) {
    const unsigned long long a = (unsigned long long)p, b = a + (unsigned)bytes;
    const unsigned long long z = (unsigned long long)isdqn_zero_block;
    if (a >= z && b <= z + sizeof(isdqn_zero_block)) return;
    const int n = isdqn_bounds.n;
    if (n <= 0) return;
    bool ok = false;
    for (int i = 0; i < n; ++i) ok |= (a >= isdqn_bounds.lo[i] && b <= isdqn_bounds.hi[i]);
    if (!ok && atomicCAS(&isdqn_bounds.bad, 0, 1) == 0) {
        isdqn_bounds.bad_addr = a;
        isdqn_bounds.bad_site = site;
    }
}
#define ISDQN_BOUNDS_CHECK(p, bytes, site) bounds_check((const void*)(p), (int)(bytes), (site))
#else
#define ISDQN_BOUNDS_CHECK(p, bytes, site) ((void)0)
#endif
__device__ __forceinline__ void mask8(bool ok, float (&v)[8]) {
#pragma unroll
    for (int i = 0; i < 8; ++i) v[i] = ok ? v[i] : 0.f;
}
#define ISDQN_GLOBAL __attribute__((address_space(1)))
__device__ __forceinline__ f32x4 nt_load4(const float* p) { return __builtin_nontemporal_load((const ISDQN_GLOBAL f32x4*)p); }
__device__ __forceinline__ void nt_store4(float* p, const f32x4& v) { __builtin_nontemporal_store(v, (ISDQN_GLOBAL f32x4*)p); }
__device__ __forceinline__ float adam_element(float& m, float& v, float p, float g, float b1, float b2, float lr, float eps, float inv_c1,
                                              float inv_c2) {
    m = b1 * m + (1.f - b1) * g;
    v = b2 * v + (1.f - b2) * g * g;
#if defined(ISDQN_ADAM_IEEE)
    return p - lr * ((m * inv_c1) / (sqrtf(v * inv_c2) + eps));
#else
    const float den = __builtin_amdgcn_sqrtf(v * inv_c2) + eps;
    return p - lr * ((m * inv_c1) * __builtin_amdgcn_rcpf(den));
#endif
}
__device__ __forceinline__ void load8_aligned(const float* p, float (&v)[8]) {
    ISDQN_BOUNDS_CHECK(p, 32, 1);
    const ISDQN_GLOBAL f32x4* gp = (const ISDQN_GLOBAL f32x4*)p;
    const f32x4 a = gp[0];
    const f32x4 b = gp[1];
    v[0] = a[0]; v[1] = a[1]; v[2] = a[2]; v[3] = a[3];
    v[4] = b[0]; v[5] = b[1]; v[6] = b[2]; v[7] = b[3];
}
__device__ __forceinline__ unsigned long long load_u64_unaligned(const uint8_t* p) {
    typedef unsigned long long __attribute__((aligned(1))) u64_u;
    ISDQN_BOUNDS_CHECK(p, 8, 2);
    return *(const ISDQN_GLOBAL u64_u*)p;
}

struct MatSrc {
    const float* base;
    int ld, outer, inner;
    int aligned8;
    template <bool ALIGNED = true>
    __device__ __forceinline__ void load(int o, int i0, float (&v)[8]) const {
        const bool ok = (o < outer) && (i0 < inner);
        if constexpr (ALIGNED) {
            load8_aligned(ok ? base + (int64_t)o * ld + i0 : zero_chunk(), v);
        } else {
            const float* p = base + (ok ? (int64_t)o * ld + i0 : (int64_t)0);
            const int last = ok ? inner - 1 - i0 : 0;
            ISDQN_BOUNDS_CHECK(p, 4 * ((last < 7 ? last : 7) + 1), 3);
#pragma unroll
            for (int j = 0; j < 8; ++j) {
                float x = p[j <= last ? j : last];
                v[j] = (ok && j <= last) ? x : 0.f;
            }
        }
    }
};

}
```

Before: 4264.

## Specialize conv forward kernels on LayerNorm and full-width channels, precompute gather offsets

Adds LN and FULL template parameters to the image and pair conv kernels so the epilogue drops runtime gamma and channel-bound checks, and moves it into a shared ConvEpilogue helper. Gather source and destination offsets are precomputed once per thread instead of being recomputed on each walk. Weight-chunk addressing becomes a compile-time-K offset, and the XCD tile mapping uses FastDiv. pin_loaded asm barriers are added to keep loads in flight ahead of use. The cost is more kernel instantiations and extra live registers for the cached offsets.

```diff
diff --git a/is-dqn_amd/build.py b/is-dqn_amd/build.py
--- a/is-dqn_amd/build.py
+++ b/is-dqn_amd/build.py
@@ -27,6 +27,8 @@
     flags = FLAGS + ["-D" + d for d in defines] + list(extra_flags)
     os.makedirs(objdir, exist_ok=True)
     headers = [os.path.join(CSRC, h) for h in HEADERS]
+    if not force and not _stale(lib, [os.path.join(CSRC, s) for s in SOURCES] + headers):
+        return lib
     objs = []
     procs = []
     for src in SOURCES:
diff --git a/is-dqn_amd/csrc/conv_img.h b/is-dqn_amd/csrc/conv_img.h
--- a/is-dqn_amd/csrc/conv_img.h
+++ b/is-dqn_amd/csrc/conv_img.h
@@ -48,6 +48,7 @@
     FastDiv d_chunk, d_Wp, d_R;
     PixelOrder order;
     long long* stamps;
+    FastDiv d_T, d_8T;
 };
 
 template <int MT, int PASSES, bool U8>
@@ -63,6 +64,102 @@
     static constexpr int A_STAGE = A_PLANES * GA::ELEMS;
 };
 
+template <int KDIM, bool ALL_ROWS>
+struct WeightChunk {
+    unsigned off;
+    const float* ptr;
+    int kmul;
+    __device__ __forceinline__ void init(const MatSrc& W, int row, int k0) {
+        if constexpr (ALL_ROWS) {
+            off = (unsigned)(row * KDIM + k0) * 4u;
+        } else {
+            const bool ok = row < W.outer;
+            ptr = ok ? W.base + (row * KDIM + k0) : zero_chunk();
+            kmul = ok ? 1 : 0;
+        }
+    }
+    __device__ __forceinline__ void load(const MatSrc& W, int k, float (&v)[8]) const {
+        if constexpr (ALL_ROWS) load8_aligned(reinterpret_cast<const float*>(reinterpret_cast<const char*>(W.base + k) + off), v);
+        else load8_aligned(ptr + k * kmul, v);
+    }
+};
+
+template <int MTW, bool LN, bool FULL>
+struct ConvEpilogue {
+    float bi[MTW][4], ga[MTW][4], be[MTW][4];
+    __device__ __forceinline__ void read_params(const float (&s_par)[3][64], int grp) {
+#pragma unroll
+        for (int mt = 0; mt < MTW; ++mt) {
+            const int ch0 = (mt * 16 + grp * 4) & 63;
+            const float4 b4 = *reinterpret_cast<const float4*>(&s_par[0][ch0]);
+            bi[mt][0] = b4.x; bi[mt][1] = b4.y; bi[mt][2] = b4.z; bi[mt][3] = b4.w;
+            if constexpr (LN) {
+                const float4 g4 = *reinterpret_cast<const float4*>(&s_par[1][ch0]);
+                const float4 e4 = *reinterpret_cast<const float4*>(&s_par[2][ch0]);
+                ga[mt][0] = g4.x; ga[mt][1] = g4.y; ga[mt][2] = g4.z; ga[mt][3] = g4.w;
+                be[mt][0] = e4.x; be[mt][1] = e4.y; be[mt][2] = e4.z; be[mt][3] = e4.w;
+            }
+        }
+    }
+    template <class AccOf>
+    __device__ __forceinline__ void tile(const ConvImgParams& p, int grp, int j, int out_pix, AccOf&& acc_of) const {
+        const ConvGeom& g = p.g;
+        const float inv_c = FULL ? 1.0f / (float)(MTW * 16) : 1.0f / (float)g.cout;
+        float zv[MTW][4], s1 = 0.f, s2 = 0.f;
+#pragma unroll
+        for (int mt = 0; mt < MTW; ++mt)
+#pragma unroll
+            for (int r = 0; r < 4; ++r) {
+                const int ch = mt * 16 + grp * 4 + r;
+                const float zz = (FULL || ch < g.cout) ? acc_of(mt, r) * p.scale + bi[mt][r] : 0.f;
+                zv[mt][r] = zz;
+                s1 += zz;
+                s2 += zz * zz;
+            }
+        float mean = 0.f, rstd = 1.f;
+        if constexpr (LN) {
+            s1 += __shfl_xor(s1, 16); s1 += __shfl_xor(s1, 32);
+            s2 += __shfl_xor(s2, 16); s2 += __shfl_xor(s2, 32);
+            mean = s1 * inv_c;
+            const float var = fmaxf(s2 * inv_c - mean * mean, 0.f);
+            rstd = rsqrtf(var + 1e-6f);
+        }
+        s8_quad_t aq[MTW];
+#pragma unroll
+        for (int mt = 0; mt < MTW; ++mt) {
+            const int ch0 = mt * 16 + grp * 4;
+            float a[4];
+#pragma unroll
+            for (int r = 0; r < 4; ++r) {
+                const float y = LN ? (zv[mt][r] - mean) * (rstd * ga[mt][r]) + be[mt][r] : zv[mt][r];
+                a[r] = (FULL || ch0 + r < g.cout) ? fmaxf(y, 0.f) : 0.f;
+            }
+            aq[mt] = s8_pack_quad_paired(a[0], a[1], a[2], a[3]);
+        }
+        const int64_t img0 = (int64_t)j * g.npix * g.cout_p;
+        char* act_img = reinterpret_cast<char*>(p.act + img0);
+        char* z_img = reinterpret_cast<char*>(p.z + img0);
+        const unsigned row = (unsigned)(out_pix * g.cout_p) * 4u;
+        const bool with_z = j < p.z_img;
+        if (out_pix >= 0) {
+#pragma unroll
+            for (int mt = 0; mt < MTW; ++mt) {
+                const int ch0 = mt * 16 + grp * 4;
+                if (!FULL && ch0 >= g.cout_p) continue;
+                *reinterpret_cast<s8_quad_t*>(act_img + (row + (unsigned)s8_quad_paired_offset(ch0) * 4u)) = aq[mt];
+            }
+            if (with_z) {
+#pragma unroll
+                for (int mt = 0; mt < MTW; ++mt) {
+                    const int ch0 = mt * 16 + grp * 4;
+                    if (!FULL && ch0 >= g.cout_p) continue;
+                    *reinterpret_cast<float4*>(z_img + (row + (unsigned)ch0 * 4u)) = make_float4(zv[mt][0], zv[mt][1], zv[mt][2], zv[mt][3]);
+                }
+            }
+        }
+    }
+};
+
 __device__ __forceinline__ void xcd_image_tile(int wg, int n_img, int T, int& j, int& tile) {
     const int full = (n_img / 8) * 8 * T;
     if (T > 1 && wg < full) {
@@ -73,6 +170,15 @@
         j = wg / T;
         tile = wg - j * T;
     }
+}
+
+__device__ __forceinline__ void xcd_image_tile(int wg, int n_img, int T, const FastDiv& d_T, const FastDiv& d_8T, int& j, int& tile) {
+    const int full = (n_img / 8) * 8 * T;
+    const bool grouped = T > 1 && wg < full;
+    const int q = (int)(grouped ? d_8T.div((uint32_t)wg) : d_T.div((uint32_t)wg));
+    const int r = wg - q * (grouped ? 8 * T : T);
+    j = grouped ? q * 8 + (r & 7) : q;
+    tile = grouped ? r >> 3 : r;
 }
 
 template <int NTHR, int PLANES, int BATCH>
@@ -220,7 +326,7 @@
 }
 
 
-template <int MT, int PASSES, bool U8, int KG = 1>
+template <int MT, int PASSES, bool U8, int KG = 1, bool LN = true>
 __global__ __launch_bounds__(GEMM_THREADS * KG, (U8 && MT == 2 && PASSES == 2) ? 4 : 1) void conv_fwd_img_kernel(const ConvImgParams p) {
     ISDQN_EMPTY_KERNEL_RETURN
     using T = ConvImgTraits<MT, PASSES, U8>;
@@ -263,7 +369,7 @@
     {
         const int which = tid >> 6, ch = tid & 63;
         const float* src = which == 0 ? p.bias : which == 1 ? p.gamma : p.beta;
-        const bool ok = kg == 0 && tid < 192 && ch < g.cout_p && src != nullptr;
+        const bool ok = kg == 0 && tid < (LN ? 192 : 64) && ch < g.cout_p && src != nullptr;
         ISDQN_BOUNDS_CHECK(ok ? src + ch : zero_chunk(), 4, 13);
         par_v = *(const ISDQN_GLOBAL float*)(ok ? src + ch : zero_chunk());
     }
@@ -508,66 +614,12 @@
         return;
     }
 
-    float bi[MTW][4], ga[MTW][4], be[MTW][4];
-#pragma unroll
-    for (int mt = 0; mt < MTW; ++mt) {
-        const int ch0 = ((mt0 + mt) * 16 + grp * 4) & 63;
-        const float4 b4 = *reinterpret_cast<const float4*>(&s_par[0][ch0]);
-        const float4 g4 = *reinterpret_cast<const float4*>(&s_par[1][ch0]);
-        const float4 e4 = *reinterpret_cast<const float4*>(&s_par[2][ch0]);
-        bi[mt][0] = b4.x; bi[mt][1] = b4.y; bi[mt][2] = b4.z; bi[mt][3] = b4.w;
-        ga[mt][0] = g4.x; ga[mt][1] = g4.y; ga[mt][2] = g4.z; ga[mt][3] = g4.w;
-        be[mt][0] = e4.x; be[mt][1] = e4.y; be[mt][2] = e4.z; be[mt][3] = e4.w;
-    }
-    const float inv_c = 1.0f / (float)g.cout;
-    float zv[NT][MTW][4], s1[NT], s2[NT];
-#pragma unroll
-    for (int nt = 0; nt < NT; ++nt) {
-        s1[nt] = s2[nt] = 0.f;
-        if (KG > 1 && nt != kg) continue;
-#pragma unroll
-        for (int mt = 0; mt < MTW; ++mt)
-#pragma unroll
-            for (int r = 0; r < 4; ++r) {
-                int ch = (mt0 + mt) * 16 + grp * 4 + r;
-                float zz = ch < g.cout ? acc[mt][nt][r] * p.scale + bi[mt][r] : 0.f;
-                zv[nt][mt][r] = zz;
-                s1[nt] += zz;
-                s2[nt] += zz * zz;
-            }
-        if (p.gamma != nullptr) {
-            s1[nt] += __shfl_xor(s1[nt], 16); s1[nt] += __shfl_xor(s1[nt], 32);
-            s2[nt] += __shfl_xor(s2[nt], 16); s2[nt] += __shfl_xor(s2[nt], 32);
-        }
-    }
+    ConvEpilogue<MTW, LN, false> epi;
+    epi.read_params(s_par, grp);
 #pragma unroll
     for (int nt = 0; nt < NT; ++nt) {
         if (KG > 1 && nt != kg) continue;
-        float mean = 0.f, rstd = 1.f;
-        if (p.gamma != nullptr) {
-            mean = s1[nt] * inv_c;
-            float var = fmaxf(s2[nt] * inv_c - mean * mean, 0.f);
-            rstd = rsqrtf(var + 1e-6f);
-        }
-        if (out_pix[nt] >= 0) {
-            const int64_t pix = (int64_t)j * g.npix + out_pix[nt];
-#pragma unroll
-            for (int mt = 0; mt < MTW; ++mt) {
-                int ch0 = (mt0 + mt) * 16 + grp * 4;
-                if (ch0 >= g.cout_p) continue;
-                float4 a, zq;
-                float* ap = &a.x;
-                float* zp = &zq.x;
-#pragma unroll
-                for (int r = 0; r < 4; ++r) {
-                    float y = p.gamma != nullptr ? (zv[nt][mt][r] - mean) * (rstd * ga[mt][r]) + be[mt][r] : zv[nt][mt][r];
-                    ap[r] = (ch0 + r < g.cout) ? fmaxf(y, 0.f) : 0.f;
-                    zp[r] = zv[nt][mt][r];
-                }
-                s8_store_quad_paired(p.act + pix * g.cout_p, ch0, a.x, a.y, a.z, a.w);
-                if (j < p.z_img) *reinterpret_cast<float4*>(p.z + pix * g.cout_p + ch0) = zq;
-            }
-        }
+        epi.tile(p, grp, j, out_pix[nt], [&](int mt, int r) { return acc[mt][nt][r]; });
     }
     ISDQN_STAMP(4);
 #if defined(ISDQN_DEV)
@@ -580,17 +632,22 @@
 #undef ISDQN_ABLATED
 }
 
-template <int MT, int PASSES, bool U8, int KG = 1>
-static int launch_conv_fwd_img(const ConvImgParams& p, hipStream_t st) {
+template <int MT, int PASSES, bool U8, int KG, bool LN>
+static int launch_conv_fwd_img_as(const ConvImgParams& p, hipStream_t st) {
     using T = ConvImgTraits<MT, PASSES, U8>;
     const int lds = (KG * 2 * T::A_STAGE + T::B_PLANES * p.plane_elems) * 2;
     static LdsConfigured configured;
-    if (int rc = ensure_dynamic_lds(&conv_fwd_img_kernel<MT, PASSES, U8, KG>, lds, configured)) return rc;
-    ISDQN_REPORT_OCCUPANCY((&conv_fwd_img_kernel<MT, PASSES, U8, KG>), GEMM_THREADS * KG, lds, p.n_img * p.tiles_per_img);
-    hipLaunchKernelGGL((conv_fwd_img_kernel<MT, PASSES, U8, KG>), dim3(p.n_img * p.tiles_per_img), dim3(GEMM_THREADS * KG), lds,
+    if (int rc = ensure_dynamic_lds(&conv_fwd_img_kernel<MT, PASSES, U8, KG, LN>, lds, configured)) return rc;
+    ISDQN_REPORT_OCCUPANCY((&conv_fwd_img_kernel<MT, PASSES, U8, KG, LN>), GEMM_THREADS * KG, lds, p.n_img * p.tiles_per_img);
+    hipLaunchKernelGGL((conv_fwd_img_kernel<MT, PASSES, U8, KG, LN>), dim3(p.n_img * p.tiles_per_img), dim3(GEMM_THREADS * KG), lds,
                        st, p);
     ISDQN_HIP_CHECK(hipGetLastError());
     return ISDQN_OK;
+}
+
+template <int MT, int PASSES, bool U8, int KG = 1>
+static int launch_conv_fwd_img(const ConvImgParams& p, hipStream_t st) {
+    return p.gamma != nullptr ? launch_conv_fwd_img_as<MT, PASSES, U8, KG, true>(p, st) : launch_conv_fwd_img_as<MT, PASSES, U8, KG, false>(p, st);
 }
 
 static inline int conv_img_geometry(const ConvGeom& g, bool u8, int stack, int b_planes, int mt, int a_planes, int& R,
diff --git a/is-dqn_amd/csrc/conv_s8_pair.h b/is-dqn_amd/csrc/conv_s8_pair.h
--- a/is-dqn_amd/csrc/conv_s8_pair.h
+++ b/is-dqn_amd/csrc/conv_s8_pair.h
@@ -5,10 +5,11 @@
 
 constexpr int S8P_BATCH = 6;
 
-template <int NPOS>
+template <int NPOS, bool LN, bool FULL>
 __global__ __launch_bounds__(GEMM_THREADS * 2, 1) void conv_fwd_s8_pair_kernel(const ConvImgParams p) {
     ISDQN_EMPTY_KERNEL_RETURN
     constexpr int MT = 4, PASSES = 3, KG = 2, NT = 2, MTW = MT, NTHR = GEMM_THREADS, NTHR_ALL = GEMM_THREADS * KG;
+    constexpr int KDIM = NPOS * KG * GEMM_BK;
     using T = ConvImgTraits<MT, PASSES, false>;
     using GA = typename T::GA;
     extern __shared__ __attribute__((aligned(16))) char smem_raw[];
@@ -25,18 +26,20 @@
     {
         const int which = tid >> 6, ch = tid & 63;
         const float* src = which == 0 ? p.bias : which == 1 ? p.gamma : p.beta;
-        const bool ok = kg == 0 && tid < 192 && ch < g.cout_p && src != nullptr;
+        const bool ok = kg == 0 && tid < (LN ? 192 : 64) && ch < g.cout_p && src != nullptr;
         ISDQN_BOUNDS_CHECK(ok ? src + ch : zero_chunk(), 4, 13);
         par_v = *(const ISDQN_GLOBAL float*)(ok ? src + ch : zero_chunk());
     }
     constexpr int nsteps = NPOS * KG;
-    const int k_last = g.K - 8;
+    constexpr int k_last = KDIM - 8;
     static_assert(GA::CHUNKS == NTHR, "one weight chunk per thread and K step");
-    const int a_row = stash_row(tid), a_var = (tid & 3) * 8, a_lds = a_row * GA::PITCH + (tid & 3) * 8;
+    const int a_row = stash_row(tid), a_lds = a_row * GA::PITCH + (tid & 3) * 8;
+    WeightChunk<KDIM, FULL> a_src;
+    a_src.init(p.W, a_row, (tid & 3) * 8);
     constexpr int PF = 4;
     static_assert(NPOS >= PF + 2, "ring of four slices + two staged ones");
     float sa[PF][1][8];
-    auto fetch = [&](int slot, int k) { p.W.load(a_row, k + a_var, sa[slot][0]); };
+    auto fetch = [&](int slot, int k) { a_src.load(p.W, k, sa[slot][0]); };
     auto stash = [&](int slot, int stage) {
         __bf16* a_hi = a_stage + stage * T::A_STAGE;
         __bf16* a_lo = a_hi + GA::ELEMS;
@@ -52,14 +55,19 @@
     p.d_Wp.divmod(dpix_u, dpy_u, dpx_u);
     const int dpix = (int)dpix_u, dcc = (int)dcc_u, dpy = (int)dpy_u, dpx = (int)dpx_u;
     float rv[S8P_BATCH][8];
-    auto walk = [&](auto&& visit) {
+    int w_src[S8P_BATCH], w_dst[S8P_BATCH];
+    {
         uint32_t pix_u, cc_u, lr_u, xl_u;
         p.d_chunk.divmod((uint32_t)tid_all, pix_u, cc_u);
         p.d_Wp.divmod(pix_u, lr_u, xl_u);
         int cc = (int)cc_u, lr = (int)lr_u, xl = (int)xl_u, pix = (int)pix_u, c0 = tid_all;
 #pragma unroll
         for (int u = 0; u < S8P_BATCH; ++u) {
-            visit(u, c0 < n_chunks, lr, xl, cc, pix);
+            const bool on = c0 < n_chunks;
+            const int iy = row_base + lr, ix = xl - g.pad;
+            const bool ok = on && iy >= 0 && iy < g.hin && ix >= 0 && ix < g.win;
+            w_src[u] = ok ? (iy * g.win + ix) * g.cin_p + cc * 8 : -1;
+            w_dst[u] = on ? pix * p.PP + cc * 8 : -1;
             c0 += NTHR_ALL;
             cc += dcc;
             const int carry_c = cc >= cpp ? 1 : 0;
@@ -71,28 +79,26 @@
             xl -= carry_x ? p.Wp : 0;
             lr += carry_x;
         }
-    };
+    }
     auto request = [&](int j) {
         const float* src = p.in + (int64_t)j * g.hin * g.win * g.cin_p;
-        walk([&](int u, bool on, int lr, int xl, int cc, int) {
-            const int iy = row_base + lr, ix = xl - g.pad;
-            const bool ok = on && iy >= 0 && iy < g.hin && ix >= 0 && ix < g.win;
-            load8_aligned(ok ? src + ((iy * g.win + ix) * g.cin_p + cc * 8) : zero_chunk(), rv[u]);
-        });
+#pragma unroll
+        for (int u = 0; u < S8P_BATCH; ++u) load8_aligned(w_src[u] >= 0 ? src + w_src[u] : zero_chunk(), rv[u]);
     };
     auto commit = [&]() {
-        walk([&](int u, bool on, int, int, int cc, int pix) {
+#pragma unroll
+        for (int u = 0; u < S8P_BATCH; ++u) {
             bf16x8 hi, lo;
+            pin_loaded(rv[u]);
             s8_unpack(rv[u], hi, lo);
-            if (on) {
-                const int dst = pix * p.PP + cc * 8;
-                *reinterpret_cast<bf16x8*>(img + p.plane_elems + dst) = lo;
-                *reinterpret_cast<bf16x8*>(img + dst) = hi;
-            }
-        });
-    };
-
-    int b_org[NT], out_pix[NT];
+            if (w_dst[u] >= 0) {
+                *reinterpret_cast<bf16x8*>(img + p.plane_elems + w_dst[u]) = lo;
+                *reinterpret_cast<bf16x8*>(img + w_dst[u]) = hi;
+            }
+        }
+    };
+
+    int b_org[NT], out_mine = -1;
 #pragma unroll
     for (int nt = 0; nt < NT; ++nt) {
         int pp = wave * 32 + nt * 16 + column_slot(lane & 15);
@@ -100,7 +106,7 @@
         pp = in_img ? pp : g.npix - 1;
         int oy, ox;
         p.order.map(pp, oy, ox);
-        out_pix[nt] = in_img ? oy * g.wout + ox : -1;
+        out_mine = nt == kg ? (in_img ? oy * g.wout + ox : -1) : out_mine;
         const int ly0 = oy * g.stride - g.pad - row_base;
         const int lx0 = ox * g.stride;
         b_org[nt] = (ly0 * p.Wp + lx0) * p.PP;
@@ -204,6 +210,7 @@
             }
             __syncthreads();
         }
+        float mine[MTW][4];
         {
             float* red = reinterpret_cast<float*>(img);
 #pragma unroll
@@ -219,87 +226,35 @@
 #pragma unroll
                 for (int r = 0; r < 4; ++r) {
                     const float got = red[((((1 - kg) * 4 + wave) * MTW + mt) * 4 + r) * 64 + lane];
-                    if (kg == 0) acc[mt][0][r] += got;
-                    else acc[mt][1][r] += got;
+                    mine[mt][r] = (kg == 0 ? acc[mt][0][r] : acc[mt][1][r]) + got;
                 }
         }
-        float bi[MTW][4], ga[MTW][4], be[MTW][4];
-#pragma unroll
-        for (int mt = 0; mt < MTW; ++mt) {
-            const int ch0 = (mt * 16 + grp * 4) & 63;
-            const float4 b4 = *reinterpret_cast<const float4*>(&s_par[0][ch0]);
-            const float4 g4 = *reinterpret_cast<const float4*>(&s_par[1][ch0]);
-            const float4 e4 = *reinterpret_cast<const float4*>(&s_par[2][ch0]);
-            bi[mt][0] = b4.x; bi[mt][1] = b4.y; bi[mt][2] = b4.z; bi[mt][3] = b4.w;
-            ga[mt][0] = g4.x; ga[mt][1] = g4.y; ga[mt][2] = g4.z; ga[mt][3] = g4.w;
-            be[mt][0] = e4.x; be[mt][1] = e4.y; be[mt][2] = e4.z; be[mt][3] = e4.w;
-        }
-        const float inv_c = 1.0f / (float)g.cout;
-        float zv[NT][MTW][4], s1[NT], s2[NT];
-#pragma unroll
-        for (int nt = 0; nt < NT; ++nt) {
-            s1[nt] = s2[nt] = 0.f;
-            if (nt != kg) continue;
-#pragma unroll
-            for (int mt = 0; mt < MTW; ++mt)
-#pragma unroll
-                for (int r = 0; r < 4; ++r) {
-                    int ch = mt * 16 + grp * 4 + r;
-                    float zz = ch < g.cout ? acc[mt][nt][r] * p.scale + bi[mt][r] : 0.f;
-                    zv[nt][mt][r] = zz;
-                    s1[nt] += zz;
-                    s2[nt] += zz * zz;
-                }
-            if (p.gamma != nullptr) {
-                s1[nt] += __shfl_xor(s1[nt], 16); s1[nt] += __shfl_xor(s1[nt], 32);
-                s2[nt] += __shfl_xor(s2[nt], 16); s2[nt] += __shfl_xor(s2[nt], 32);
-            }
-        }
-#pragma unroll
-        for (int nt = 0; nt < NT; ++nt) {
-            if (nt != kg) continue;
-            float mean = 0.f, rstd = 1.f;
-            if (p.gamma != nullptr) {
-                mean = s1[nt] * inv_c;
-                float var = fmaxf(s2[nt] * inv_c - mean * mean, 0.f);
-                rstd = rsqrtf(var + 1e-6f);
-            }
-            if (out_pix[nt] >= 0) {
-                const int64_t pix = (int64_t)j * g.npix + out_pix[nt];
-#pragma unroll
-                for (int mt = 0; mt < MTW; ++mt) {
-                    int ch0 = mt * 16 + grp * 4;
-                    if (ch0 >= g.cout_p) continue;
-                    float4 a, zq;
-                    float* ap = &a.x;
-                    float* zp = &zq.x;
-#pragma unroll
-                    for (int r = 0; r < 4; ++r) {
-                        float y = p.gamma != nullptr ? (zv[nt][mt][r] - mean) * (rstd * ga[mt][r]) + be[mt][r] : zv[nt][mt][r];
-                        ap[r] = (ch0 + r < g.cout) ? fmaxf(y, 0.f) : 0.f;
-                        zp[r] = zv[nt][mt][r];
-                    }
-                    s8_store_quad_paired(p.act + pix * g.cout_p, ch0, a.x, a.y, a.z, a.w);
-                    if (j < p.z_img) *reinterpret_cast<float4*>(p.z + pix * g.cout_p + ch0) = zq;
-                }
-            }
-        }
+        ConvEpilogue<MTW, LN, FULL> epi;
+        epi.read_params(s_par, grp);
+        epi.tile(p, grp, j, out_mine, [&](int mt, int r) { return mine[mt][r]; });
         if constexpr (it == 0) __syncthreads();
     };
     do_image(std::integral_constant<int, 0>{});
     do_image(std::integral_constant<int, 1>{});
 }
 
-template <int NPOS>
-static int launch_conv_fwd_s8_pair(const ConvImgParams& p, hipStream_t st) {
+template <int NPOS, bool LN, bool FULL>
+static int launch_conv_fwd_s8_pair_as(const ConvImgParams& p, hipStream_t st) {
     using T = ConvImgTraits<4, 3, false>;
     const int lds = (2 * 2 * T::A_STAGE + T::B_PLANES * p.plane_elems) * 2;
     static LdsConfigured configured;
-    if (int rc = ensure_dynamic_lds(&conv_fwd_s8_pair_kernel<NPOS>, lds, configured)) return rc;
-    ISDQN_REPORT_OCCUPANCY((&conv_fwd_s8_pair_kernel<NPOS>), GEMM_THREADS * 2, lds, p.n_img / 2);
-    hipLaunchKernelGGL((conv_fwd_s8_pair_kernel<NPOS>), dim3(p.n_img / 2), dim3(GEMM_THREADS * 2), lds, st, p);
+    if (int rc = ensure_dynamic_lds(&conv_fwd_s8_pair_kernel<NPOS, LN, FULL>, lds, configured)) return rc;
+    ISDQN_REPORT_OCCUPANCY((&conv_fwd_s8_pair_kernel<NPOS, LN, FULL>), GEMM_THREADS * 2, lds, p.n_img / 2);
+    hipLaunchKernelGGL((conv_fwd_s8_pair_kernel<NPOS, LN, FULL>), dim3(p.n_img / 2), dim3(GEMM_THREADS * 2), lds, st, p);
     ISDQN_HIP_CHECK(hipGetLastError());
     return ISDQN_OK;
 }
 
-}
+template <int NPOS>
+static int launch_conv_fwd_s8_pair(const ConvImgParams& p, hipStream_t st) {
+    const bool ln = p.gamma != nullptr, full = p.g.cout == 64 && p.g.cout_p == 64;
+    if (ln) return full ? launch_conv_fwd_s8_pair_as<NPOS, true, true>(p, st) : launch_conv_fwd_s8_pair_as<NPOS, true, false>(p, st);
+    return full ? launch_conv_fwd_s8_pair_as<NPOS, false, true>(p, st) : launch_conv_fwd_s8_pair_as<NPOS, false, false>(p, st);
+}
+
+}
diff --git a/is-dqn_amd/csrc/conv_u8_pair.h b/is-dqn_amd/csrc/conv_u8_pair.h
--- a/is-dqn_amd/csrc/conv_u8_pair.h
+++ b/is-dqn_amd/csrc/conv_u8_pair.h
@@ -5,10 +5,10 @@
 
 constexpr int U8P_PB = 2;
 
-template <int PASSES, int NSTEPS>
+template <int PASSES, int NSTEPS, bool LN, bool FULL>
 __global__ __launch_bounds__(GEMM_THREADS, 4) void conv_fwd_u8_pair_kernel(const ConvImgParams p) {
     ISDQN_EMPTY_KERNEL_RETURN
-    constexpr int MT = 2, NT = 2, MTW = MT, NTHR = GEMM_THREADS, STACK_MAX = 4;
+    constexpr int MT = 2, NT = 2, MTW = MT, NTHR = GEMM_THREADS, STACK = 4, KDIM = NSTEPS * GEMM_BK;
     using T = ConvImgTraits<MT, PASSES, true>;
     using GA = typename T::GA;
     extern __shared__ __attribute__((aligned(16))) char smem_raw[];
@@ -29,36 +29,37 @@
     U8P_STAMP(0);
     const int T2 = p.tiles_per_img >> 1;
     int j, tp;
-    xcd_image_tile((int)blockIdx.x, p.n_img, T2, j, tp);
+    xcd_image_tile((int)blockIdx.x, p.n_img, T2, p.d_T, p.d_8T, j, tp);
 
     __shared__ __attribute__((aligned(16))) float s_par[3][64];
     float par_v = 0.f;
     {
         const int which = tid >> 6, ch = tid & 63;
         const float* src = which == 0 ? p.bias : which == 1 ? p.gamma : p.beta;
-        const bool ok = tid < 192 && ch < g.cout_p && src != nullptr;
+        const bool ok = tid < (LN ? 192 : 64) && ch < g.cout_p && src != nullptr;
         ISDQN_BOUNDS_CHECK(ok ? src + ch : zero_chunk(), 4, 13);
         par_v = *(const ISDQN_GLOBAL float*)(ok ? src + ch : zero_chunk());
     }
     constexpr int nsteps = NSTEPS;
-    const int k_last = g.K - 8;
+    constexpr int k_last = KDIM - 8;
     constexpr int A_PER = (GA::CHUNKS + NTHR - 1) / NTHR;
-    int a_row[A_PER], a_var[A_PER], a_lds[A_PER];
+    int a_lds[A_PER];
     bool a_on[A_PER];
+    WeightChunk<KDIM, FULL> a_src[A_PER];
 #pragma unroll
     for (int i = 0; i < A_PER; ++i) {
         int c = tid + i * NTHR;
         a_on[i] = c < GA::CHUNKS;
         if (!a_on[i]) c = 0;
-        a_row[i] = stash_row(c);
-        a_var[i] = (c & 3) * 8;
-        a_lds[i] = a_row[i] * GA::PITCH + (c & 3) * 8;
+        const int a_row = stash_row(c);
+        a_src[i].init(p.W, a_row, (c & 3) * 8);
+        a_lds[i] = a_row * GA::PITCH + (c & 3) * 8;
     }
     constexpr int PF = 4;
     float sa[PF][A_PER][8];
     auto fetch = [&](int slot, int k) {
 #pragma unroll
-        for (int i = 0; i < A_PER; ++i) p.W.load(a_row[i], k + a_var[i], sa[slot][i]);
+        for (int i = 0; i < A_PER; ++i) a_src[i].load(p.W, k, sa[slot][i]);
     };
     auto stash = [&](int slot, int stage) {
         __bf16* a_hi = a_stage + stage * T::A_STAGE;
@@ -79,48 +80,56 @@
     static_assert(NSTEPS >= PF + 2 && NSTEPS % 2 == 0, "ring of four slices + two staged ones");
 
     const FrameSrc& fs = p.fs;
-    const uint8_t* base[STACK_MAX];
-#pragma unroll
-    for (int c = 0; c < STACK_MAX; ++c) {
-        const int id = c < fs.stack ? fs.frame_id(j, c) : -1;
-        base[c] = id >= 0 ? fs.frames + (int64_t)id * fs.stride : nullptr;
-    }
-    const uint8_t* zeros = reinterpret_cast<const uint8_t*>(zero_chunk());
+    const uint8_t* base[STACK];
+    bool have[STACK];
+#pragma unroll
+    for (int c = 0; c < STACK; ++c) {
+        const int id = __builtin_amdgcn_readfirstlane(fs.frame_id(j, c));
+        have[c] = id >= 0;
+        base[c] = fs.frames + (int64_t)(have[c] ? id : 0) * fs.stride;
+    }
     const int cpr = p.Wp / 8, per_plane = p.R * cpr, plane = p.R * p.Wp;
-    unsigned long long raw[U8P_PB][STACK_MAX];
+    constexpr int ROW_OFF = 1 << 28;
+    int q_row[U8P_PB], q_off[U8P_PB], q_sh[U8P_PB], q_dst[U8P_PB];
+#pragma unroll
+    for (int k = 0; k < U8P_PB; ++k) {
+        const int pos = k * NTHR + tid;
+        const bool on = pos < per_plane;
+        uint32_t lr, cx;
+        p.d_chunk.divmod((uint32_t)(on ? pos : 0), lr, cx);
+        const int ix0 = (int)cx * 8 - g.pad;
+        const int ixc = min(max(ix0, 0), fs.W - 8);
+        q_row[k] = (on && ix0 > -8 && ix0 < fs.W) ? (int)lr : ROW_OFF;
+        q_off[k] = (int)lr * fs.W + ixc;
+        q_sh[k] = ix0 - ixc;
+        q_dst[k] = on ? (int)lr * p.Wp + (int)cx * 8 : -1;
+    }
+    unsigned long long raw[U8P_PB][STACK];
     auto request = [&](int row_base) {
 #pragma unroll
         for (int k = 0; k < U8P_PB; ++k) {
-            const int pos = k * NTHR + tid;
-            const bool on = pos < per_plane;
-            uint32_t lr, cx;
-            p.d_chunk.divmod((uint32_t)(on ? pos : 0), lr, cx);
-            const int iy = row_base + (int)lr, ix0 = (int)cx * 8 - g.pad;
-            const bool ok = on && iy >= 0 && iy < fs.H && ix0 > -8 && ix0 < fs.W;
-            const int ixc = min(max(ix0, 0), fs.W - 8);
-            const int off = iy * fs.W + ixc;
-#pragma unroll
-            for (int c = 0; c < STACK_MAX; ++c) raw[k][c] = load_u64_unaligned((ok && base[c] != nullptr) ? base[c] + off : zeros);
-        }
-    };
-    auto commit = [&]() {
+            const bool ok = (unsigned)(row_base + q_row[k]) < (unsigned)fs.H;
+            const unsigned off = ok ? (unsigned)(row_base * fs.W + q_off[k]) : 0u;
+#pragma unroll
+            for (int c = 0; c < STACK; ++c) raw[k][c] = load_u64_unaligned(base[c] + off);
+        }
+    };
+    auto commit = [&](int row_base) {
 #pragma unroll
         for (int k = 0; k < U8P_PB; ++k) {
-            const int pos = k * NTHR + tid;
-            const bool on = pos < per_plane;
-            uint32_t lr, cx;
-            p.d_chunk.divmod((uint32_t)(on ? pos : 0), lr, cx);
-            const int ix0 = (int)cx * 8 - g.pad;
-            const int sh = ix0 - min(max(ix0, 0), fs.W - 8);
-            const int dst = (int)lr * p.Wp + (int)cx * 8;
-#pragma unroll
-            for (int c = 0; c < STACK_MAX; ++c) {
-                if (c >= fs.stack) continue;
+            const bool ok = (unsigned)(row_base + q_row[k]) < (unsigned)fs.H;
+            bf16x8 hi[STACK];
+#pragma unroll
+            for (int c = 0; c < STACK; ++c) pin_loaded(raw[k][c]);
+#pragma unroll
+            for (int c = 0; c < STACK; ++c) {
                 float v[8];
-                FrameSrc::patch8_cvt(raw[k][c], sh, v);
-                bf16x8 hi;
-                round8(v, hi);
-                if (on) *reinterpret_cast<bf16x8*>(img + c * plane + dst) = hi;
+                FrameSrc::patch8_cvt((ok && have[c]) ? raw[k][c] : 0ull, q_sh[k], v);
+                round8(v, hi[c]);
+            }
+            if (q_dst[k] >= 0) {
+#pragma unroll
+                for (int c = 0; c < STACK; ++c) *reinterpret_cast<bf16x8*>(img + c * plane + q_dst[k]) = hi[c];
             }
         }
     };
@@ -148,7 +157,7 @@
 #pragma unroll
         for (int d = 0; d < PF; ++d) fetch(d, slice(d) * GEMM_BK);
         if constexpr (it == 0) request(row_base);
-        commit();
+        commit(row_base);
         U8P_STAMP(it == 0 ? 1 : 4);
 
         int b_org[NT], out_pix[NT];
@@ -232,65 +241,10 @@
         }
 
         U8P_STAMP(it == 0 ? 2 : 5);
-        float bi[MTW][4], ga[MTW][4], be[MTW][4];
-#pragma unroll
-        for (int mt = 0; mt < MTW; ++mt) {
-            const int ch0 = (mt * 16 + grp * 4) & 63;
-            const float4 b4 = *reinterpret_cast<const float4*>(&s_par[0][ch0]);
-            const float4 g4 = *reinterpret_cast<const float4*>(&s_par[1][ch0]);
-            const float4 e4 = *reinterpret_cast<const float4*>(&s_par[2][ch0]);
-            bi[mt][0] = b4.x; bi[mt][1] = b4.y; bi[mt][2] = b4.z; bi[mt][3] = b4.w;
-            ga[mt][0] = g4.x; ga[mt][1] = g4.y; ga[mt][2] = g4.z; ga[mt][3] = g4.w;
-            be[mt][0] = e4.x; be[mt][1] = e4.y; be[mt][2] = e4.z; be[mt][3] = e4.w;
-        }
-        const float inv_c = 1.0f / (float)g.cout;
-        float zv[NT][MTW][4], s1[NT], s2[NT];
-#pragma unroll
-        for (int nt = 0; nt < NT; ++nt) {
-            s1[nt] = s2[nt] = 0.f;
-#pragma unroll
-            for (int mt = 0; mt < MTW; ++mt)
-#pragma unroll
-                for (int r = 0; r < 4; ++r) {
-                    int ch = mt * 16 + grp * 4 + r;
-                    float zz = ch < g.cout ? acc[mt][nt][r] * p.scale + bi[mt][r] : 0.f;
-                    zv[nt][mt][r] = zz;
-                    s1[nt] += zz;
-                    s2[nt] += zz * zz;
-                }
-            if (p.gamma != nullptr) {
-                s1[nt] += __shfl_xor(s1[nt], 16); s1[nt] += __shfl_xor(s1[nt], 32);
-                s2[nt] += __shfl_xor(s2[nt], 16); s2[nt] += __shfl_xor(s2[nt], 32);
-            }
-        }
-#pragma unroll
-        for (int nt = 0; nt < NT; ++nt) {
-            float mean = 0.f, rstd = 1.f;
-            if (p.gamma != nullptr) {
-                mean = s1[nt] * inv_c;
-                float var = fmaxf(s2[nt] * inv_c - mean * mean, 0.f);
-                rstd = rsqrtf(var + 1e-6f);
-            }
-            if (out_pix[nt] >= 0) {
-                const int64_t pix = (int64_t)j * g.npix + out_pix[nt];
-#pragma unroll
-                for (int mt = 0; mt < MTW; ++mt) {
-                    int ch0 = mt * 16 + grp * 4;
-                    if (ch0 >= g.cout_p) continue;
-                    float4 a, zq;
-                    float* ap = &a.x;
-                    float* zp = &zq.x;
-#pragma unroll
-                    for (int r = 0; r < 4; ++r) {
-                        float y = p.gamma != nullptr ? (zv[nt][mt][r] - mean) * (rstd * ga[mt][r]) + be[mt][r] : zv[nt][mt][r];
-                        ap[r] = (ch0 + r < g.cout) ? fmaxf(y, 0.f) : 0.f;
-                        zp[r] = zv[nt][mt][r];
-                    }
-                    s8_store_quad_paired(p.act + pix * g.cout_p, ch0, a.x, a.y, a.z, a.w);
-                    if (j < p.z_img) *reinterpret_cast<float4*>(p.z + pix * g.cout_p + ch0) = zq;
-                }
-            }
-        }
+        ConvEpilogue<MTW, LN, FULL> epi;
+        epi.read_params(s_par, grp);
+#pragma unroll
+        for (int nt = 0; nt < NT; ++nt) epi.tile(p, grp, j, out_pix[nt], [&](int mt, int r) { return acc[mt][nt][r]; });
         U8P_STAMP(it == 0 ? 3 : 6);
     };
     do_tile(std::integral_constant<int, 0>{});
@@ -298,17 +252,27 @@
 #undef U8P_STAMP
 }
 
-template <int PASSES, int NSTEPS>
-static int launch_conv_fwd_u8_pair(const ConvImgParams& p, hipStream_t st) {
+template <int PASSES, int NSTEPS, bool LN, bool FULL>
+static int launch_conv_fwd_u8_pair_as(const ConvImgParams& p, hipStream_t st) {
     using T = ConvImgTraits<2, PASSES, true>;
     const int lds = (2 * T::A_STAGE + T::B_PLANES * p.plane_elems) * 2;
     static LdsConfigured configured;
-    if (int rc = ensure_dynamic_lds(&conv_fwd_u8_pair_kernel<PASSES, NSTEPS>, lds, configured)) return rc;
+    if (int rc = ensure_dynamic_lds(&conv_fwd_u8_pair_kernel<PASSES, NSTEPS, LN, FULL>, lds, configured)) return rc;
     const int grid = p.n_img * (p.tiles_per_img / 2);
-    ISDQN_REPORT_OCCUPANCY((&conv_fwd_u8_pair_kernel<PASSES, NSTEPS>), GEMM_THREADS, lds, grid);
-    hipLaunchKernelGGL((conv_fwd_u8_pair_kernel<PASSES, NSTEPS>), dim3(grid), dim3(GEMM_THREADS), lds, st, p);
+    ISDQN_REPORT_OCCUPANCY((&conv_fwd_u8_pair_kernel<PASSES, NSTEPS, LN, FULL>), GEMM_THREADS, lds, grid);
+    hipLaunchKernelGGL((conv_fwd_u8_pair_kernel<PASSES, NSTEPS, LN, FULL>), dim3(grid), dim3(GEMM_THREADS), lds, st, p);
     ISDQN_HIP_CHECK(hipGetLastError());
     return ISDQN_OK;
 }
 
-}
+template <int PASSES, int NSTEPS>
+static int launch_conv_fwd_u8_pair(const ConvImgParams& p_in, hipStream_t st) {
+    ConvImgParams p = p_in;
+    p.d_T = FastDiv((uint32_t)(p.tiles_per_img / 2));
+    p.d_8T = FastDiv((uint32_t)(8 * (p.tiles_per_img / 2)));
+    const bool ln = p.gamma != nullptr, full = p.g.cout == 32 && p.g.cout_p == 32;
+    if (ln) return full ? launch_conv_fwd_u8_pair_as<PASSES, NSTEPS, true, true>(p, st) : launch_conv_fwd_u8_pair_as<PASSES, NSTEPS, true, false>(p, st);
+    return full ? launch_conv_fwd_u8_pair_as<PASSES, NSTEPS, false, true>(p, st) : launch_conv_fwd_u8_pair_as<PASSES, NSTEPS, false, false>(p, st);
+}
+
+}
diff --git a/is-dqn_amd/csrc/gemm_core.h b/is-dqn_amd/csrc/gemm_core.h
--- a/is-dqn_amd/csrc/gemm_core.h
+++ b/is-dqn_amd/csrc/gemm_core.h
@@ -75,10 +75,10 @@
     *reinterpret_cast<bf16x4*>(g + 16) = lo;
 }
 
-__device__ __forceinline__ void s8_store_quad_paired(float* row, int c0, float v0, float v1, float v2, float v3) {
+typedef __attribute__((ext_vector_type(4))) unsigned s8_quad_t;
+__device__ __forceinline__ s8_quad_t s8_pack_quad_paired(float v0, float v1, float v2, float v3) {
     typedef __attribute__((ext_vector_type(4))) __bf16 bf16x4;
     typedef __attribute__((ext_vector_type(2))) unsigned u32x2;
-    typedef __attribute__((ext_vector_type(4))) unsigned u32x4;
     const float v[4] = {v0, v1, v2, v3};
     bf16x4 hi, lo;
 #pragma unroll
@@ -90,8 +90,11 @@
     const u32x2 h = __builtin_bit_cast(u32x2, hi), l = __builtin_bit_cast(u32x2, lo);
     const auto r0 = __builtin_amdgcn_permlane16_swap(h[0], l[0], false, false);
     const auto r1 = __builtin_amdgcn_permlane16_swap(h[1], l[1], false, false);
-    char* g = reinterpret_cast<char*>(row + (c0 & ~7)) + (c0 & 4) * 4;
-    *reinterpret_cast<u32x4*>(g) = u32x4{r0[0], r1[0], r0[1], r1[1]};
+    return s8_quad_t{r0[0], r1[0], r0[1], r1[1]};
+}
+__device__ __forceinline__ int s8_quad_paired_offset(int c0) { return (c0 & ~7) + (c0 & 4); }
+__device__ __forceinline__ void s8_store_quad_paired(float* row, int c0, float v0, float v1, float v2, float v3) {
+    *reinterpret_cast<s8_quad_t*>(row + s8_quad_paired_offset(c0)) = s8_pack_quad_paired(v0, v1, v2, v3);
 }
 
 __device__ __forceinline__ void s8_store_pair(float* row, int c0, float v0, float v1) {
@@ -429,6 +432,10 @@
     return p - lr * ((m * inv_c1) * __builtin_amdgcn_rcpf(den));
 #endif
 }
+__device__ __forceinline__ void pin_loaded(unsigned long long& v) { asm volatile("" : "+v"(v)); }
+__device__ __forceinline__ void pin_loaded(float (&v)[8]) {
+    asm volatile("" : "+v"(v[0]), "+v"(v[1]), "+v"(v[2]), "+v"(v[3]), "+v"(v[4]), "+v"(v[5]), "+v"(v[6]), "+v"(v[7]));
+}
 __device__ __forceinline__ void load8_aligned(const float* p, float (&v)[8]) {
     ISDQN_BOUNDS_CHECK(p, 32, 1);
     const ISDQN_GLOBAL f32x4* gp = (const ISDQN_GLOBAL f32x4*)p;
```

After: 4286 (median of 2 runs). About the same (+0.5%).
